# loro-dev/loro

Hardware: AMD Instinct MI355X
Metric: merged docs/sec (batch of N docs x M remote ops) (higher is better)
Workload: dtype u32; 1 GPU; configs[1]: 10000 docs/GPU x 100000-op automerge-paper-shaped text trace, 2 concurrent peers, 3 FastUpdates blobs/doc (4683 op runs, 30 changes, 103435 blob bytes/doc); docs_per_gpu=10000, ops_per_doc=100000, contexts_in_flight=2, streams_per_context=2

## Files before the change

loro_amd/csrc/lm_k_decode.h:

```cpp
#pragma once
#include "lm_dev_util.h"

namespace lm {

struct Dev {
  const uint8_t* data;
  const uint64_t* blob_off;
  const uint32_t* blob_len;
  const uint32_t* doc_blob;
  uint32_t n_blobs, n_docs;
  uint32_t span;
  const uint32_t* res_old_blobs;
  uint32_t loc_cleared;
  uint32_t* posdel;
  const uint64_t* posdel_off;
  uint32_t* pd_row_idx;
  const uint8_t* vvo;
  const uint64_t* vvo_off;
  const uint8_t* doc_fused;
  uint32_t n_op_rows;
  uint32_t* blk_kind;
  uint32_t posdel_redo;
  uint32_t no_linear;
  uint32_t res_vis;
  const uint8_t* front;
  const uint64_t* front_off;
  const uint8_t* froot;
  const uint64_t* froot_off;
  int32_t* blob_status;
  uint32_t* blob_hash;
  uint32_t* blob_nblk;
  uint32_t* blob_blk0;
  uint32_t* blob_doc;
  uint32_t n_blocks;
  BlockDesc* blk;
  uint32_t* bcnt;
  uint32_t* boff;
  ChangeRow* chg;
  uint32_t* dep_peer;
  uint32_t* dep_ctr;
  uint32_t* dep_ci;
  OpRow* op;
  uint64_t* op_val;
  uint32_t* op_blk;
  uint64_t* key_off;
  uint32_t* key_len;
  uint32_t* cid_raw;
  uint32_t* cid_map;
  uint64_t* peer_raw;
  uint32_t* peer_map;
  DocMeta* doc;
  const uint32_t* doc_order;
  uint64_t* peer_uniq;
  uint32_t* peer_end;
  uint32_t* peer_ext;
  uint32_t* peer_base;
  uint32_t* peer_end_all;
  uint32_t* elem_base;
  uint32_t* elem_cap;
  uint32_t* peer_chg0;
  uint32_t* peer_chg1;
  ContRow* cont;
  uint32_t* chg_sorted;
  uint32_t* chg_lamport;
  uint32_t* chg_skip;
  uint32_t* chg_flag;
  uint32_t* chg_mask;
  uint32_t* node_first;
  uint32_t* node_last;
  uint32_t* node_order;
  uint32_t* vvh;
  uint32_t* cp;
  uint32_t* loc;
  uint32_t* dcnt;
  uint8_t* tb;
  uint32_t* it;
  uint8_t* lf_chunk;
  uint32_t* dir_out;
  uint32_t* cont_root0;
  uint32_t* cont_nroot;
  unsigned long long* ht_key;
  unsigned long long* ht_best;
  unsigned long long* ht_pfx;
  uint64_t* ht0;
  uint32_t* ht_cap;
  uint32_t* ht_list;
  uint32_t* ht_cnt;
  unsigned long long* prof;
  uint32_t* fuse;
  uint32_t* dec_stat;
  uint32_t dec_slot;
  uint32_t vs_row_cost;
  uint32_t cut_min_rows;
  uint8_t* out;
  uint64_t* out_off;
  uint8_t* vv_out;
  uint64_t* vv_off;
};
static constexpr int BCN = 8;
enum { BC_CHG = 0, BC_DEP, BC_OP, BC_KEY, BC_CID, BC_PEER, BC_MAPOP, BC_ATOMS };
static constexpr uint32_t VIS_CAP = 1024;
static constexpr uint32_t TB_WIDE = 0xFF, TB_ANCHOR = 0xFE;
static constexpr uint32_t CP_ANCHOR = 0x80000000u, CP_ALIVE = 0x40000000u;

static constexpr uint64_t BIG_BLOB = 32768;
static constexpr uint32_t HASH_G = 4;
LM_DEV uint32_t xx_round(uint32_t v, uint32_t m) { return rotl32(v + m, 13) * 0x9E3779B1u; }
LM_KERNEL LM_WAVES_PER_SIMD(2) LM_ONE_WAVE_GROUPS void k_hash_big_blobs(Dev d, const uint32_t* big, uint32_t n_big) {
  const uint32_t P1 = 0x9E3779B1u, P2 = 0x85EBCA77u, P3 = 0xC2B2AE3Du, P4 = 0x27D4EB2Fu, P5 = 0x165667B1u;
  const uint32_t seed = 0x4f524f4cu;
  uint32_t lane = (uint32_t)lmw::lane(), row = lane >> 4, rl = lane & 15, a = lane & 3;
  uint32_t i = (uint32_t)lmw::bid() * HASH_G + row;
  bool have = i < n_big;
  uint32_t b = big[have ? i : 0u];
  uint64_t blen = have ? d.blob_len[b] : 0ull;
  uint64_t len = blen >= 1024 + 20 ? blen - 20 : 0ull;
  const uint8_t* p = d.data + d.blob_off[b] + 20;
  const uint32_t* w = (const uint32_t*)p + rl;
  uint32_t v = a == 0 ? seed + P1 + P2 : a == 1 ? seed + P2 : a == 2 ? seed : seed - P1;
  const uint32_t n_str = (uint32_t)(len >> 4), n_kb = n_str >> 6;
  const uint32_t T = lmw::reduce_max(n_kb);
  uint32_t xa[16], xb[16], xc[16];
  const uint32_t kb_last = n_kb ? n_kb - 1 : 0u;
#define LM_HASH_LOAD(x, t) do { const uint32_t* q_ = w + (size_t)256 * ((t) < kb_last ? (t) : kb_last); _Pragma("unroll") for (int k_ = 0; k_ < 16; k_++) x[k_] = q_[16 * k_]; } while (0)
#define LM_HASH_CHAIN(x, t) do { uint32_t nv_ = v; _Pragma("unroll") for (int k_ = 0; k_ < 16; k_++) { const uint32_t m_ = x[k_] * P2; \
      nv_ = xx_round(nv_, m_); nv_ = xx_round(nv_, lmw::row_down<4>(m_)); nv_ = xx_round(nv_, lmw::row_down<8>(m_)); nv_ = xx_round(nv_, lmw::row_down<12>(m_)); LM_SCHED_FENCE(); } \
    if ((t) < n_kb) v = nv_; } while (0)
  LM_HASH_LOAD(xa, 0u); LM_HASH_LOAD(xb, 1u);
#pragma unroll 1
  for (uint32_t t = 0; t < T; t += 3) {
    LM_HASH_LOAD(xc, t + 2); LM_HASH_CHAIN(xa, t);
    LM_HASH_LOAD(xa, t + 3); LM_HASH_CHAIN(xb, t + 1);
    LM_HASH_LOAD(xb, t + 4); LM_HASH_CHAIN(xc, t + 2);
  }
#undef LM_HASH_LOAD
#undef LM_HASH_CHAIN
  {
    const uint32_t s0 = n_kb << 6;
#pragma unroll 1
    for (uint32_t c = 0; c < 16; c++) {
      const uint32_t s_ = s0 + 4 * c;
      const uint32_t st_ = s_ + (rl >> 2), stc_ = st_ < n_str ? st_ : (n_str ? n_str - 1 : 0u);
      const uint32_t x = ((const uint32_t*)p)[(size_t)4 * stc_ + a];
      const uint32_t m_ = x * P2;
      uint32_t nv = xx_round(v, m_);
      if (s_ < n_str) v = nv;
      nv = xx_round(v, lmw::row_down<4>(m_));
      if (s_ + 1 < n_str) v = nv;
      nv = xx_round(v, lmw::row_down<8>(m_));
      if (s_ + 2 < n_str) v = nv;
      nv = xx_round(v, lmw::row_down<12>(m_));
      if (s_ + 3 < n_str) v = nv;
    }
  }
  int g0 = (int)(lane & ~15u);
  uint32_t v1 = lmw::shfl(v, g0), v2 = lmw::shfl(v, g0 + 1), v3 = lmw::shfl(v, g0 + 2), v4 = lmw::shfl(v, g0 + 3);
  uint32_t h = rotl32(v1, 1) + rotl32(v2, 7) + rotl32(v3, 12) + rotl32(v4, 18);
  h += (uint32_t)len;
  const uint8_t* q = p + ((uint64_t)n_str << 4);
  const uint8_t* end = p + len;
  while (q + 4 <= end) { h = rotl32(h + ld32le(q) * P3, 17) * P4; q += 4; }
  while (q < end) { h = rotl32(h + (*q) * P5, 11) * P1; q++; }
  h ^= h >> 15; h *= P2; h ^= h >> 13; h *= P3; h ^= h >> 16;
  if (have && rl == 0) d.blob_hash[b] = len >= 16 ? h : 0u;
}

LM_KERNEL void k_frame_count(Dev d) {
  uint32_t b = (uint32_t)(lmw::bid() * lmw::bdim() + lmw::tid());
  if (b >= d.n_blobs) return;
  const uint8_t* p = d.data + d.blob_off[b];
  uint64_t len = d.blob_len[b];
  int32_t st = ST_OK;
  uint32_t nblk = 0;
  if (len < 22) st = ST_DECODE_ERROR;
  else if (!(p[0] == 'l' && p[1] == 'o' && p[2] == 'r' && p[3] == 'o')) st = ST_DECODE_ERROR;
  else {
    uint32_t mode = ((uint32_t)p[20] << 8) | p[21];
    if (mode == 3) st = ST_UNSUPPORTED;
    else if (mode != 4) st = ST_DECODE_ERROR;
    else {
      uint32_t expect = ld32le(p + 16);
      uint32_t h = len >= BIG_BLOB ? d.blob_hash[b] : xxh32_lane(p + 20, len - 20, 0x4f524f4cu);
      if (h != expect) st = ST_CHECKSUM_MISMATCH;
      else {
        Rd r = rd_make(p + 22, len - 22);
        while (r.p < r.end && !r.bad) {
          uint64_t bl = rd_uleb(r);
          if (bl == 0 || bl > rd_left(r)) { r.bad = true; break; }
          r.p += bl;
          nblk++;
        }
        if (r.bad) { st = ST_DECODE_ERROR; nblk = 0; }
      }
    }
  }
  d.blob_status[b] = st;
  d.blob_nblk[b] = nblk;
}

LM_KERNEL void k_frame_fill(Dev d) {
  uint32_t b = (uint32_t)(lmw::bid() * lmw::bdim() + lmw::tid());
  if (b >= d.n_blobs) return;
  if (d.blob_status[b] != ST_OK) return;
  uint64_t base = d.blob_off[b];
  const uint8_t* p = d.data + base;
  uint64_t len = d.blob_len[b];
  Rd r = rd_make(p + 22, len - 22);
  uint32_t bi = d.blob_blk0[b];
  uint32_t nblk = d.blob_nblk[b];
  uint32_t doc = d.blob_doc[b];
  for (uint32_t k = 0; k < nblk; k++, bi++) {
    uint64_t bl = rd_uleb(r);
    BlockDesc* o = d.blk + bi;
    o->base = (uint64_t)(r.p - d.data);
    o->blob = b;
    o->doc = doc;
    o->pad = (uint32_t)bl;
    r.p += bl;
  }
}
LM_KERNEL void k_block_desc(Dev d) {
  uint32_t bi = (uint32_t)(lmw::bid() * lmw::bdim() + lmw::tid());
  if (bi >= d.n_blocks) return;
  BlockDesc bd = d.blk[bi];
  const uint8_t* p0 = d.data + bd.base;
  Rd q = rd_make(p0, bd.pad);
// ... 553 lines not shown
```

loro_amd/csrc/lm_k_integrate_span.h:

```cpp
#pragma once
#include "lm_k_integrate.h"

namespace lm {

static constexpr uint32_t SP_REC = 320;
LM_DEV uint32_t sa_make(uint32_t leaf, uint32_t n, bool nf) { return leaf | (nf ? DIR_NF : 0u) | (n << 18); }
LM_DEV uint32_t sa_leaf(uint32_t a) { return a & DIR_LEAF_MASK; }
LM_DEV uint32_t sa_n(uint32_t a) { return (a >> 18) & 0x7f; }
LM_DEV bool sa_nf(uint32_t a) { return (a & DIR_NF) != 0; }

struct SpanRegs { uint32_t n, id, len, ol, orr, st; };
struct SpanItem { uint32_t id, len, ol, orr, st; };

struct Ts {
  uint32_t* it;
  uint32_t* loc;
  const uint32_t* ebase;
  const uint32_t* cur;
  const uint32_t* end;
  uint32_t* da;
  uint32_t* db;
  uint32_t* ds;
  bool ds_on;
  uint32_t n_dir, dir_cap, n_leaf, leaf_cap, tot_active;
  uint32_t n_alive;
  uint32_t cache_leaf;
  uint32_t cache_p;
  uint32_t cache_pre;
  SpanRegs cr;
  bool dirty;
  uint32_t loc_pend;
  int32_t err;
  uint32_t beyond;
#ifdef LM_PROF
  mutable uint64_t prof[PF_N];
#endif
};
static constexpr int32_t ST_POSDEL = 101;
static constexpr uint32_t PD_CAP = 63;
static constexpr uint32_t PD_LDS = 12;
LM_DEV uint32_t* pd_w(const Ts& t) { return const_cast<uint32_t*>(t.ebase) - PD_LDS; }
template <bool POS>
LM_DEV void pd_stop(Ts& t, uint32_t k, uint32_t left, uint32_t first, uint32_t matched) {
#ifdef LM_EMU_TRACE
  if (getenv("LM_EMU_BASE") && lmw::lane() == 0 && t.err) fprintf(stderr, "pd_stop<%d> with err %d\n", (int)POS, (int)t.err);
#endif
  if (!POS || t.err != ST_RETRY) t.err = ST_POSDEL;
  if (POS && lmw::lane() == 0) { uint32_t* w = pd_w(t); w[0] = k; w[1] = left; w[2] = first; w[3] = matched; }
}

LM_DEV uint32_t ts_g(const Ts& t, uint32_t pid) { return t.ebase[pid_peer(pid)] + pid_ctr(pid); }
LM_DEV bool sp_has(uint32_t id0, uint32_t len, uint32_t x) { return x >= id0 && x - id0 < len; }

LM_DEV SpanRegs sp_load(const Ts& t, uint32_t L, uint32_t n) {
  int lane = lmw::lane();
  lmw::wave_sync();
  if (L == t.cache_leaf) return t.cr;
  PROF_CNT(t, PF_NEXTRA, 1);
  SpanRegs r;
  r.n = n;
  bool in = (uint32_t)lane < n;
  const uint32_t* rec = t.it + (uint64_t)L * SP_REC;
  r.id = in ? rec[lane] : NONE;
  r.len = in ? rec[64 + lane] : 0u;
  r.ol = in ? rec[128 + lane] : NONE;
  r.orr = in ? rec[192 + lane] : NONE;
  r.st = in ? rec[256 + lane] : ST_FUT;
  return r;
}
LM_DEV void sp_write(Ts& t, uint32_t L, const SpanRegs& R) {
  int lane = lmw::lane();
  if ((uint32_t)lane < R.n) {
    uint32_t* rec = t.it + (uint64_t)L * SP_REC;
    rec[lane] = R.id; rec[64 + lane] = R.len; rec[128 + lane] = R.ol; rec[192 + lane] = R.orr; rec[256 + lane] = R.st;
  }
}
LM_DEV uint32_t sp_alen(const SpanRegs& R) { return st_active(R.st) ? R.len : 0u; }
LM_DEV bool sp_nf(const SpanRegs& R) { return lmw::ballot(!(R.st & ST_FUT)) != 0; }
LM_DEV uint64_t sp_hit(const SpanRegs& R, uint32_t x) { return lmw::ballot(x - R.id < R.len); }
#ifndef LM_LOC_SHORT
#define LM_LOC_SHORT 16
#endif
static constexpr uint32_t LOC_SHORT = LM_LOC_SHORT;
#if !defined(LM_LOC_FULL) && !defined(LM_LOC16)
#define LM_LOC16 1
#endif
#ifdef LM_LOC16
#ifndef LM_LOC_W
#define LM_LOC_W 64
#endif
static constexpr uint32_t LOC_W = LM_LOC_W;
LM_DEV void sp_set_loc_lanes(Ts& t, const SpanRegs& R, bool pend, uint32_t L) {
  if (!t.loc) return;
  uint32_t len = pend ? R.len : 0u;
  uint32_t c0 = pid_ctr(R.id);
  uint32_t g = pend ? t.ebase[pid_peer(R.id)] + c0 : 0u;
  if (pend) t.loc[g] = L;
  uint32_t k = LOC_W - (c0 & (LOC_W - 1));
  for (uint32_t i = 0; i < 4 && lmw::any(k < len); i++, k += LOC_W) if (k < len) t.loc[g + k] = L;
  uint64_t m = lmw::ballot(k < len);
  while (m) {
    int j = lmw::ffs64(m);
    m &= m - 1;
    uint32_t gj = lmw::bcast(g, j), lj = lmw::bcast(len, j), kj = lmw::bcast(k, j);
    for (uint32_t kk = kj + LOC_W * (uint32_t)lmw::lane(); kk < lj; kk += 64 * LOC_W) t.loc[gj + kk] = L;
  }
}
LM_DEV uint32_t ts_loc_find(const Ts& t, uint32_t pid) {
  if (!t.loc) return NONE;
  uint32_t ctr = pid_ctr(pid), lo = ctr & ~(LOC_W - 1), eb = t.ebase[pid_peer(pid)];
  uint32_t lane = (uint32_t)lmw::lane();
  uint32_t v = (lane < LOC_W && lo + lane <= ctr) ? t.loc[eb + lo + lane] : NONE;
  uint64_t m = lmw::ballot(v != NONE);
  if (!m) return NONE;
  int top = 63 - __builtin_clzll((unsigned long long)m);
  return lmw::bcast(v, top);
}
#else
LM_DEV void sp_set_loc_lanes(Ts& t, const SpanRegs& R, bool pend, uint32_t L) {
  uint32_t len = pend ? R.len : 0u;
  uint32_t g = pend ? t.ebase[pid_peer(R.id)] + pid_ctr(R.id) : 0u;
  uint32_t lim = len < LOC_SHORT ? len : LOC_SHORT;
  for (uint32_t k = 0; k < lim; k++) t.loc[g + k] = L;
  uint64_t m = lmw::ballot(len > LOC_SHORT);
  while (m) {
    int j = lmw::ffs64(m);
    m &= m - 1;
    uint32_t gj = lmw::bcast(g, j), lj = lmw::bcast(len, j);
    for (uint32_t k = LOC_SHORT + (uint32_t)lmw::lane(); k < lj; k += 64) t.loc[gj + k] = L;
  }
}
#endif
LM_DEV void sp_flush(Ts& t) {
  if (t.cache_leaf == NONE) return;
  if (t.dirty) { sp_write(t, t.cache_leaf, t.cr); t.dirty = false; }
  if (lmw::any(t.loc_pend != 0)) { sp_set_loc_lanes(t, t.cr, t.loc_pend != 0, t.cache_leaf); t.loc_pend = 0; }
}
LM_DEV void sp_flush_loc(Ts& t) {
  if (t.cache_leaf != NONE && lmw::any(t.loc_pend != 0)) { sp_set_loc_lanes(t, t.cr, t.loc_pend != 0, t.cache_leaf); t.loc_pend = 0; }
}
LM_DEV void sd_sync_cached(Ts& t);
LM_DEV void sp_take(Ts& t, uint32_t L) {
  if (t.cache_leaf != L) { sp_flush(t); sd_sync_cached(t); t.cache_leaf = L; t.dirty = false; t.loc_pend = 0; }
}

#ifndef LM_SD_LINEAR
#define LM_SD_LINEAR 128
#endif
static constexpr uint32_t SD_LINEAR = LM_SD_LINEAR;
#ifndef LM_SD_BSH
#define LM_SD_BSH 6
#endif
static constexpr uint32_t SD_BSH = LM_SD_BSH, SD_BS = 1u << LM_SD_BSH;
LM_DEV void sd_block_sum(Ts& t, uint32_t j) {
  uint32_t i = (j << SD_BSH) + (uint32_t)lmw::lane();
  lmw::wave_sync();
  uint32_t s = lmw::reduce_add(((uint32_t)lmw::lane() < SD_BS && i < t.n_dir) ? t.db[i] : 0u);
  if (lmw::lane() == 0) t.ds[j] = s;
  lmw::wave_sync();
}
LM_DEV void sd_sums_from(Ts& t, uint32_t j0) { for (uint32_t j = j0; (j << SD_BSH) < t.n_dir; j++) sd_block_sum(t, j); }
LM_DEV void sd_sync_cached(Ts& t) { if (t.ds_on && t.cache_leaf != NONE && t.cache_p < t.n_dir) sd_block_sum(t, t.cache_p >> SD_BSH); }
LM_DEV void sd_set(Ts& t, uint32_t p, uint32_t a, uint32_t b) {
  lmw::wave_sync();
  uint32_t old = t.db[p];
  lmw::wave_sync();
  if (lmw::lane() == 0) { t.da[p] = a; t.db[p] = b; if (t.ds_on) t.ds[p >> SD_BSH] += b - old; }
  t.tot_active += b - old;
  lmw::wave_sync();
}
LM_DEV void sd_insert_after(Ts& t, uint32_t p, uint32_t a, uint32_t b) {
  int lane = lmw::lane();
  if (t.n_dir >= t.dir_cap) { LM_SETERR(t.err, ST_RETRY); return; }
  lmw::wave_sync();
  uint32_t q = p + 1;
  for (uint32_t hi = t.n_dir; hi > q;) {
    uint32_t c0 = hi > q + 64 ? hi - 64 : q;
    uint32_t i = c0 + (uint32_t)lane;
    bool in = i < hi;
    uint32_t va = in ? t.da[i] : 0u, vb = in ? t.db[i] : 0u;
    lmw::wave_sync();
    if (in) { t.da[i + 1] = va; t.db[i + 1] = vb; }
    lmw::wave_sync();
    hi = c0;
  }
  if (lane == 0) { t.da[q] = a; t.db[q] = b; }
  t.n_dir++;
  t.tot_active += b;
  if (t.cache_leaf != NONE && t.cache_p >= q) t.cache_p++;
  lmw::wave_sync();
  if (!t.ds_on && t.n_dir > SD_LINEAR) { t.ds_on = true; sd_sums_from(t, 0); }
  else if (t.ds_on) sd_sums_from(t, q >> SD_BSH);
}
LM_DEV uint32_t sd_find_kth(Ts& t, uint32_t& k) {
  int lane = lmw::lane();
  lmw::wave_sync();
  uint32_t first = 0;
  if (t.ds_on) {
    sd_sync_cached(t);
    uint32_t nb = (t.n_dir + SD_BS - 1) >> SD_BSH, blk = NONE;
    for (uint32_t j0 = 0; j0 < nb && blk == NONE; j0 += 64) {
      uint32_t j = j0 + (uint32_t)lane;
      uint32_t a = j < nb ? t.ds[j] : 0u;
      uint32_t inc = lmw::scan_incl_add(a);
      uint64_t m = lmw::ballot(inc >= k);
      if (m) { int s2 = lmw::ffs64(m); k -= lmw::bcast(inc, s2) - lmw::bcast(a, s2); blk = j0 + (uint32_t)s2; }
      else k -= lmw::bcast(inc, 63);
    }
    if (blk == NONE) return NONE;
    first = blk << SD_BSH;
  }
  for (uint32_t i0 = first; i0 < t.n_dir; i0 += 64) {
    uint32_t i = i0 + (uint32_t)lane;
    uint32_t a = i < t.n_dir ? t.db[i] : 0u;
    uint32_t inc = lmw::scan_incl_add(a);
    uint64_t m = lmw::ballot(inc >= k);
    if (m) {
      int s = lmw::ffs64(m);
      k -= lmw::bcast(inc, s) - lmw::bcast(a, s);
      return i0 + (uint32_t)s;
    }
    k -= lmw::bcast(inc, 63);
  }
  return NONE;
}
LM_DEV uint32_t sd_find_leaf(const Ts& t, uint32_t L) {
  int lane = lmw::lane();
  lmw::wave_sync();
  for (uint32_t i0 = 0; i0 < t.n_dir; i0 += 64) {
    uint32_t i = i0 + (uint32_t)lane;
    uint64_t m = lmw::ballot(i < t.n_dir && sa_leaf(t.da[i]) == L);
    if (m) return i0 + (uint32_t)lmw::ffs64(m);
  }
  return NONE;
}
LM_DEV uint32_t sd_prefix(Ts& t, uint32_t p) {
  int lane = lmw::lane();
  lmw::wave_sync();
  uint32_t acc = 0, first = 0;
  if (t.ds_on) {
    sd_sync_cached(t);
    uint32_t nbp = p >> SD_BSH;
    for (uint32_t j = (uint32_t)lane; j < nbp; j += 64) acc += t.ds[j];
    first = nbp << SD_BSH;
  }
  for (uint32_t i0 = first; i0 < p; i0 += 64) {
    uint32_t i = i0 + (uint32_t)lane;
    acc += i < p ? t.db[i] : 0u;
  }
  return lmw::reduce_add(acc);
}
LM_DEV bool ts_del_pos_ok(Ts& t, const SpanRegs& R, uint32_t slot, uint32_t s_off, uint32_t st0, uint32_t hint_k) {
  if (t.cache_pre == NONE) t.cache_pre = sd_prefix(t, t.cache_p);
  uint32_t al = sp_alen(R);
  uint32_t inc = lmw::scan_incl_add(al);
  uint32_t before = lmw::bcast(inc, (int)slot) - lmw::bcast(al, (int)slot);
  return st_active(st0) && t.cache_pre + before + s_off + 1 == hint_k;
}
LM_DEV void sd_refresh(Ts& t, uint32_t p, uint32_t L, const SpanRegs& R) {
  sd_set(t, p, sa_make(L, R.n, sp_nf(R)), lmw::reduce_add(sp_alen(R)));
}

LM_DEV SpanRegs sp_shift_in(const SpanRegs& R, uint32_t& lp, uint32_t idx, const SpanItem& A, const SpanItem& B, uint32_t cnt, bool setA, bool setB) {
  uint32_t lane = (uint32_t)lmw::lane();
  SpanRegs N;
  N.n = R.n + cnt;
// ... 830 lines not shown
    U4* c4 = (U4*)dcnt;
    const U4 zero4 = {0, 0, 0, 0};
    for (uint32_t i = (uint32_t)lane; i < (m.atoms + 3) / 4; i += 64) c4[i] = zero4;
  }
  lmw::mem_fence();
  lmw::wave_sync();
  for (uint32_t i0 = 0; i0 < m.n_op; i0 += 64) {
    uint32_t i = i0 + (uint32_t)lane;
    uint32_t g0 = 0, n = 0;
    if (i < m.n_op) {
      const OpRow& r = d.op[m.op0 + i];
      uint32_t ck = r.cidx_kind;
      if ((ck & 0xffff) == cidx && ((ck >> 16) & 0xff) == OK_DEL && (d.chg_flag[r.chg] & 1u)) {
        const ChangeRow& ch = d.chg[r.chg];
        uint32_t peer = ch.peer;
        uint32_t lo = ch.ctr + d.chg_skip[r.chg], hi = ts_vs_target(vv, ov_peer, ov, peer);
        if (lo < r.ctr) lo = r.ctr;
        if (hi > r.ctr + r.len) hi = r.ctr + r.len;
        if (lo < hi && r.a0 < P) {
          uint32_t a = lo - r.ctr, b = hi - r.ctr;
          uint32_t Ln = (uint32_t)(r.a2 < 0 ? -r.a2 : r.a2);
          uint32_t t0, t1;
          if (r.a2 > 0) { t0 = r.a1 + a; t1 = r.a1 + b; }
          else { t0 = r.a1 + (Ln - b); t1 = r.a1 + (Ln - a); }
          uint32_t e = t.end[r.a0];
          if (t1 > e) t1 = e;
          if (t0 < t1 && b <= Ln) { g0 = t.ebase[r.a0] + t0; n = t1 - t0; }
        }
      }
    }
    for (uint32_t k = 0; k < n && k < 16; k++) lmw::atomic_add(&dcnt[g0 + k], 1u);
    uint64_t lm_ = lmw::ballot(n > 16);
    while (lm_) {
      int src = lmw::ffs64(lm_);
      lm_ &= lm_ - 1;
      uint32_t bg = lmw::bcast(g0, src), bn = lmw::bcast(n, src);
      for (uint32_t k = 16 + (uint32_t)lane; k < bn; k += 64) lmw::atomic_add(&dcnt[bg + k], 1u);
    }
  }
  lmw::mem_fence();
  lmw::wave_sync();
  for (uint32_t q = 0; q < t.n_dir; q++) {
    uint32_t a = lmw::first(t.da[q]);
    uint32_t L = sa_leaf(a), n = sa_n(a);
    uint32_t* rec = t.it + (uint64_t)L * SP_REC;
    bool in = (uint32_t)lane < n;
    uint32_t id = in ? rec[lane] : 0u, ln = in ? rec[64 + lane] : 0u, st = in ? rec[256 + lane] : ST_FUT;
    uint32_t st1 = st;
    bool over = false, ragged = false;
    if (in) {
      uint32_t peer = pid_peer(id), ctr = pid_ctr(id);
      uint32_t cnt = dcnt[t.ebase[peer] + ctr];
      over = cnt > 0x7fffu;
      if (over) cnt = 0x7fffu;
      st1 = (st & ~(ST_FUT | ST_DELMASK)) | (ctr >= ts_vs_target(vv, ov_peer, ov, peer) ? ST_FUT : 0u) | (cnt << 8) | (cnt ? ST_EVER : 0u);
#ifdef LM_EMU_CHECK
      for (uint32_t k = 1; k < ln; k++)
        if (dcnt[t.ebase[peer] + ctr + k] != cnt || ((ctr + k >= ts_vs_target(vv, ov_peer, ov, peer)) != ((st1 & ST_FUT) != 0))) {
          fprintf(stderr, "CHECK version sweep: item %u:%u+%u is not uniform at element %u (count %u vs %u)\n", peer, ctr, ln, k, dcnt[t.ebase[peer] + ctr + k], cnt);
          ragged = true;
        }
#endif
    }
    if (lmw::any(over)) { LM_SETERR(t.err, ST_UNSUPPORTED); return; }
    if (lmw::any(ragged)) { LM_SETERR(t.err, ST_INTERNAL); return; }
    if (!lmw::any(in && st1 != st)) continue;
    if (in && st1 != st) rec[256 + lane] = st1;
    uint32_t act = lmw::reduce_add((in && st_active(st1)) ? ln : 0u);
    bool nf = lmw::ballot(in && !(st1 & ST_FUT)) != 0;
    sd_set(t, q, sa_make(L, n, nf), act);
  }
}
LM_DEV bool ts_sweep_pays(const Ts& t, const DocMeta& m, uint32_t P, const uint32_t* vv, uint32_t ov_peer, uint32_t ov, const uint32_t* s_cur) {
  uint32_t dist = 0;
  for (uint32_t p = (uint32_t)lmw::lane(); p < P; p += 64) { uint32_t c = s_cur[p], g = ts_vs_target(vv, ov_peer, ov, p); dist += c > g ? c - g : g - c; }
  dist = lmw::reduce_add(dist);
#ifdef LM_SWEEP_EAGER
  return dist > 0;
#else
  return dist > 256 && (uint64_t)dist * 16 > (uint64_t)m.atoms / 32 + m.n_op + 40ull * t.n_dir + 2048;
#endif
}
LM_DEV bool ts_sweep_pays_batch(const Ts& t, const Dev& d, const DocMeta& m, uint32_t P, const uint32_t* vv, const uint32_t* s_cur) {
  uint32_t dist = 0, np = 0;
  for (uint32_t p = (uint32_t)lmw::lane(); p < P; p += 64) { uint32_t c = s_cur[p], g = vv[p]; dist += c > g ? c - g : g - c; np += c != g ? 1u : 0u; }
  dist = lmw::reduce_add(dist);
  np = lmw::reduce_add(np);
#ifdef LM_SWEEP_EAGER
  return dist > 0;
#else
  const uint64_t rows = (uint64_t)dist * m.n_op / (m.atoms ? m.atoms : 1u);
  return dist > 16 && rows * d.vs_row_cost > 5ull * m.n_op / 4 + m.atoms / 40 + 60ull * t.n_dir + 600ull * np + 500;
#endif
}
#ifndef LM_BATCH_VSWEEP
#define LM_BATCH_VSWEEP 0
#endif
template <bool ML, bool SWEEP, bool VS, bool POS = false>
LM_DEV void ts_goto(Ts& t, const Dev& d, const DocMeta& m, uint32_t cidx, uint32_t P, const uint32_t* vv, uint32_t* s_cur, uint32_t* s_base,
                    bool& base_on, bool conv, uint32_t* loc_real, uint32_t* dcnt_real) {
  int lane = lmw::lane();
  if (!t.loc) {
    bool mv = false;
    for (uint32_t p = (uint32_t)lane; p < P; p += 64) mv |= s_cur[p] != vv[p];
    if (conv || lmw::any(mv)) ts_build_loc(t, loc_real);
  }
  bool reset = false;
  if (base_on) {
    bool same = true;
    uint32_t back = 0;
    for (uint32_t p = (uint32_t)lane; p < P; p += 64) { uint32_t v = vv[p], c = s_cur[p]; same &= v == s_base[p]; back += c > v ? c - v : 0u; }
    back = lmw::reduce_add(back);
#ifdef LM_SWEEP_EAGER
    reset = !lmw::any(!same) && back > 0;
#else
    reset = !lmw::any(!same) && back > 4 * t.n_dir + 32;
#endif
  }
#ifdef LM_EMU_TRACE
  if (getenv("LM_EMU_BASE") && lane == 0) fprintf(stderr, "BASE cont %u: %s%s (n_dir %u)\n", cidx, reset ? "reset" : "move", conv ? " +convert" : "", t.n_dir);
#endif
  if (reset) ts_reset_to_base(t, s_base);
  else if (VS && !base_on && !conv && dcnt_real && (lmw::block_sync(), ts_sweep_pays_batch(t, d, m, P, vv, s_cur))) ts_sweep_version(t, d, m, cidx, P, vv, NONE, 0, s_cur, dcnt_real);
  else
    for (uint32_t p = 0; p < P && !t.err; p++) {
      uint32_t cur = s_cur[p], tgt = vv[p];
      if (cur > tgt) ts_move_ops<ML, SWEEP, POS>(t, d, m, cidx, p, tgt, cur, -1);
      else if (cur < tgt) ts_move_ops<ML, SWEEP, POS>(t, d, m, cidx, p, cur, tgt, +1);
    }
  lmw::block_sync();
  for (uint32_t p = (uint32_t)lane; p < P; p += 64) { s_cur[p] = vv[p]; if (conv) s_base[p] = vv[p]; }
  if (conv && !t.err) { ts_convert_base(t); base_on = true; }
  lmw::block_sync();
}

#ifdef LM_EMU_CHECK
inline bool ts_check(Ts& t, const char* what, uint32_t row) {
  bool ok = true;
  sp_flush(t);
  lmw::wave_sync();
  if (lmw::lane() == 0) {
    uint32_t tot = 0;
    for (uint32_t q = 0; q < t.n_dir && ok; q++) {
      uint32_t a = t.da[q], L = sa_leaf(a), n = sa_n(a), act = 0;
      bool nf = false;
      const uint32_t* rec = t.it + (uint64_t)L * SP_REC;
      for (uint32_t i = 0; i < n; i++) {
        uint32_t id0 = rec[i], ln = rec[64 + i], st = rec[256 + i];
        if (ln == 0) { fprintf(stderr, "CHECK %s row=%u: dir[%u] leaf %u item %u has length 0\n", what, row, q, L, i); ok = false; }
        if (st_active(st)) act += ln;
        nf |= !(st & ST_FUT);
        for (uint32_t k = 0; k < ln && t.loc; k++) {
#ifdef LM_LOC16
          uint32_t expect = (k == 0 || ((id0 + k) & (LOC_W - 1)) == 0) ? L : NONE;
#else
          uint32_t expect = L;
#endif
          if (t.loc[ts_g(t, id0 + k)] != expect) { fprintf(stderr, "CHECK %s row=%u: loc of %u:%u is %u, item lives in leaf %u\n", what, row, id0 >> 24, (id0 & 0xffffff) + k, t.loc[ts_g(t, id0 + k)], L); ok = false; break; }
        }
      }
      if (act != t.db[q] || nf != sa_nf(a)) { fprintf(stderr, "CHECK %s row=%u: dir[%u] leaf %u active %u (cached %u) nf %d (cached %d)\n", what, row, q, L, act, t.db[q], (int)nf, (int)sa_nf(a)); ok = false; }
      tot += act;
    }
    if (ok && t.ds_on)
      for (uint32_t j = 0; (j << SD_BSH) < t.n_dir && ok; j++) {
        if (t.cache_leaf != NONE && j == (t.cache_p >> SD_BSH)) continue;
        uint32_t sum = 0;
        for (uint32_t q = j << SD_BSH; q < ((j + 1) << SD_BSH) && q < t.n_dir; q++) sum += t.db[q];
        if (sum != t.ds[j]) { fprintf(stderr, "CHECK %s row=%u: block %u sums to %u, cached sum %u\n", what, row, j, sum, t.ds[j]); ok = false; }
      }
    if (ok && tot != t.tot_active) { fprintf(stderr, "CHECK %s row=%u: total active %u, cached %u\n", what, row, tot, t.tot_active); ok = false; }
    if (ok && t.cache_leaf != NONE) {
      if (t.cache_p >= t.n_dir || sa_leaf(t.da[t.cache_p]) != t.cache_leaf) { fprintf(stderr, "CHECK %s row=%u: cached leaf %u is not at directory position %u\n", what, row, t.cache_leaf, t.cache_p); ok = false; }
      uint32_t pre = 0;
      for (uint32_t q = 0; q < t.cache_p && q < t.n_dir; q++) pre += t.db[q];
      if (ok && t.cache_pre != NONE && pre != t.cache_pre) { fprintf(stderr, "CHECK %s row=%u: %u active elements before the cached leaf, cached prefix %u\n", what, row, pre, t.cache_pre); ok = false; }
    }
  }
  return lmw::any(!ok) ? false : true;
}
#define TS_CHECK(what, row) do { if (!t.err && !ts_check(t, what, row)) t.err = ST_INTERNAL; } while (0)
#else
#define TS_CHECK(what, row) do {} while (0)
#endif

}
#include "lm_k_integrate_linear.h"
namespace lm {

struct ResDoc {
  uint64_t tk_off;
  uint32_t pcap, ccap;
  uint32_t reset;
  uint32_t elem_cap;
};
struct DevRes {
  const ResDoc* doc;
  uint32_t* tk;
  const uint32_t* dir_a_prev;
  const uint32_t* dir_b_prev;
  uint32_t* dir_b;
};
static constexpr uint32_t TK_HDR = 12, TK_CW = 8;
LM_DEV uint32_t tk_words(uint32_t pcap, uint32_t ccap) { return TK_HDR + 5 * pcap + ccap * (TK_CW + pcap); }
LM_DEV uint32_t* tk_peers(uint32_t* tk) { return tk + TK_HDR; }
LM_DEV uint32_t* tk_applied(uint32_t* tk, uint32_t pcap) { return tk + TK_HDR + 2 * pcap; }
LM_DEV uint32_t* tk_ebase(uint32_t* tk, uint32_t pcap) { return tk + TK_HDR + 3 * pcap; }
LM_DEV uint32_t* tk_ecap(uint32_t* tk, uint32_t pcap) { return tk + TK_HDR + 4 * pcap; }
LM_DEV uint32_t* tk_cont(uint32_t* tk, uint32_t pcap, uint32_t c) { return tk + TK_HDR + 5 * pcap + c * (TK_CW + pcap); }

#ifndef LM_INTEGRATE_WAVES
#define LM_INTEGRATE_WAVES 5
#endif
#if defined(LM_LOC_FULL) && !defined(LM_LAZY_LOC)
#define LM_LAZY_LOC 0
#endif
#ifndef LM_LAZY_LOC
#define LM_LAZY_LOC 1
#endif
#ifndef LM_BASE_RESET
#define LM_BASE_RESET 1
#endif
template <bool ML, bool PLAIN, bool SWEEP = false, bool RES = false, bool FUSE = false, bool POS = false>
LM_DEV void integrate_span_body(Dev d, DevDag g, uint32_t dir_cap, uint32_t pmax, const OpRow* __restrict__ op_ro,
                                const ChangeRow* __restrict__ chg_ro, const uint32_t* __restrict__ sorted_ro,
                                const uint32_t* __restrict__ skip_ro, const uint32_t* __restrict__ vvh_ro, uint32_t retry_pass,
                                uint32_t* retry_count, DevRes rs = DevRes{}) {
  uint32_t doc = d.doc_order[(uint32_t)lmw::bid()];
  int lane = lmw::lane();
  LM_DYN_SHARED(uint32_t, s_mem);
  uint32_t* s_da = s_mem;
  uint32_t* s_db = s_mem + dir_cap;
  uint32_t* s_ds = s_db + dir_cap;
  uint32_t* s_ebase = s_ds + ((dir_cap >> SD_BSH) + 2) + PD_LDS;
  uint32_t* s_cur = s_ebase + pmax;
  uint32_t* s_end = s_cur + pmax;
  uint32_t* s_tgt = s_end + pmax;
  uint32_t* s_app = s_tgt + pmax;
  uint32_t* s_pmap = s_app + pmax;
  DocMeta m = d.doc[doc];
  if (RES) {
    uint32_t* mw = (uint32_t*)&m;
    for (uint32_t i = 0; i < sizeof(DocMeta) / 4; i++) mw[i] = lmw::first(mw[i]);
  }
  uint64_t elem0 = ((uint64_t)m.elem0_hi << 32) | m.elem0_lo;
  {
    uint32_t fl = m.flags;
    if (RES && (fl & DF_PLAIN) && d.front_off[doc + 1] > d.front_off[doc]) fl &= ~DF_PLAIN;
    if (POS ? ((fl & DF_MOVABLE) != 0 || ((fl & DF_PLAIN) != 0) != PLAIN) : (fl & (DF_MOVABLE | DF_PLAIN)) != ((ML ? DF_MOVABLE : 0u) | (PLAIN ? DF_PLAIN : 0u))) return;
    if (PLAIN && !RES && !POS && ((fl & DF_FUSED) != 0 && d.fuse != nullptr) != FUSE) return;
  }
  (void)SWEEP;
  if (retry_pass && m.status != (POS ? ST_POSDEL : ST_RETRY)) return;
  if (status_fatal(m.status) && !retry_pass) return;
  const bool keep_loc = RES && !ML && !retry_pass && (m.flags & DF_LAYOUT_SAME) != 0;
  {
    struct alignas(16) U4 { uint32_t x, y, z, w; };
    U4* l4 = (U4*)(d.loc + elem0);
    const U4 none4 = {NONE, NONE, NONE, NONE};
    uint32_t from4 = 0;
    if (keep_loc) from4 = lmw::first((rs.tk + rs.doc[doc].tk_off)[6]) / 4;
    if (RES || !d.loc_cleared || retry_pass)
      for (uint32_t i = from4 + (uint32_t)lane; i < (m.atoms + 3) / 4; i += 64) l4[i] = none4;
  }
  if (retry_pass) {
    for (uint32_t c = (uint32_t)lane; c < m.n_cont; c += 64) {
      uint32_t ck = d.cont[m.cid0 + c].kind_root & 0xff;
      if (ck == CK_TEXT || ck == CK_LIST || (ML && ck == CK_MOVABLE)) d.cont[m.cid0 + c].touched = 0;
    }
    lmw::block_sync();
    if (lane == 0) d.doc[doc].status = ST_OK;
    m.status = ST_OK;
    lmw::block_sync();
  }
  if (status_fatal(m.status)) return;
  uint32_t P = m.n_peers;
  for (uint32_t p = (uint32_t)lane; p < P; p += 64) { s_ebase[p] = d.elem_base[m.praw0 + p]; s_end[p] = d.peer_end[m.praw0 + p]; }
  if (POS && !RES) for (uint32_t p = (uint32_t)lane; p < P; p += 64) s_app[p] = d.peer_base[m.praw0 + p];
  uint32_t* tk = nullptr;
  uint32_t tk_pcap = 0, P0 = 0, C0 = 0;
  bool fresh = true, renumber = false;
  const bool to_version = RES && !PLAIN && d.front_off[doc + 1] > d.front_off[doc] && !(m.flags & DF_FRONT_ERR);
  if (RES) {
    ResDoc rd;
    {
      const uint32_t* rw = (const uint32_t*)(rs.doc + doc);
      rd.tk_off = ((uint64_t)lmw::first(rw[1]) << 32) | lmw::first(rw[0]);
      rd.pcap = lmw::first(rw[2]); rd.ccap = lmw::first(rw[3]); rd.reset = lmw::first(rw[4]); rd.elem_cap = lmw::first(rw[5]);
    }
    tk = rs.tk + rd.tk_off;
    tk_pcap = rd.pcap;
    if (P > pmax || P > rd.pcap || m.n_cont > rd.ccap) { if (lane == 0) { LM_SETERR(d.doc[doc].status, ST_INTERNAL); tk[0] = 0; } return; }
    for (uint32_t p = (uint32_t)lane; p < P; p += 64) { s_tgt[p] = d.peer_end[m.praw0 + p]; s_end[p] = d.peer_end_all[m.praw0 + p]; s_app[p] = 0; }
    lmw::block_sync();
    P0 = lmw::first(tk[1]); C0 = lmw::first(tk[2]);
    fresh = rd.reset != 0 || retry_pass != 0 || lmw::first(tk[0]) != 1u || P0 > P || C0 > m.n_cont || P0 > rd.pcap;
    if (!fresh) {
      bool lost = false;
      for (uint32_t q = (uint32_t)lane; q < P0; q += 64) {
        uint64_t id = ((uint64_t)tk_peers(tk)[2 * q + 1] << 32) | tk_peers(tk)[2 * q];
        uint32_t lo = 0, hi = P;
        while (lo < hi) { uint32_t mid = (lo + hi) >> 1; if (d.peer_uniq[m.praw0 + mid] < id) lo = mid + 1; else hi = mid; }
        bool ok = lo < P && d.peer_uniq[m.praw0 + lo] == id;
        s_pmap[q] = ok ? lo : 0u;
        lost |= !ok;
        renumber |= ok && lo != q;
        if (ML && ok && tk_ebase(tk, tk_pcap)[q] != d.elem_base[m.praw0 + lo]) lost = true;
      }
      if (ML && (lmw::first(tk[4]) != m.elem0_lo || lmw::first(tk[5]) != m.elem0_hi)) lost = true;
      fresh = lmw::any(lost);
      renumber = lmw::any(renumber);
      lmw::block_sync();
      if (!fresh) for (uint32_t q = (uint32_t)lane; q < P0; q += 64) s_app[s_pmap[q]] = tk_applied(tk, tk_pcap)[q];
    }
    if (lane == 0) tk[0] = 0;
    if (fresh && !retry_pass && lane == 0) lmw::atomic_add(retry_count + 1, 1u);
  }
  lmw::block_sync();
  uint64_t vvh0 = ((uint64_t)m.vvh0_hi << 32) | m.vvh0_lo;
  Ts t;
  t.it = d.it + (uint64_t)m.leaf0 * SP_REC;
  t.loc = d.loc + elem0;
  t.ebase = s_ebase; t.cur = s_cur; t.end = s_end; t.da = s_da; t.db = s_db; t.ds = s_ds; t.ds_on = false;
  t.dir_cap = dir_cap; t.leaf_cap = m.leaf_cap; t.n_leaf = 0; t.err = 0; t.beyond = 0;
  t.n_alive = 0;
  if (lane == 0) {
    uint64_t pl = 0, ri = 0, pcap = PD_CAP;
    if (POS && d.posdel) {
      const uint64_t p0 = d.posdel_off ? d.posdel_off[doc] : (uint64_t)doc * PD_CAP;
      if (d.posdel_off) pcap = d.posdel_off[doc + 1] - p0;
      pl = (uint64_t)(uintptr_t)(d.posdel + p0 * 3);
      if (d.pd_row_idx && pcap > PD_CAP) ri = (uint64_t)(uintptr_t)d.pd_row_idx;
    }
    uint32_t* w = s_ebase - PD_LDS;
    w[0] = w[1] = w[2] = w[3] = w[4] = 0; w[5] = (uint32_t)pl; w[6] = (uint32_t)(pl >> 32);
    w[7] = (uint32_t)(pcap > 0xffffffffull ? 0xffffffffull : pcap); w[8] = (uint32_t)ri; w[9] = (uint32_t)(ri >> 32); w[10] = w[11] = 0;
  }
#ifdef LM_PROF
  for (int i = 0; i < PF_N; i++) t.prof[i] = 0;
  uint64_t pf_begin = lmw::clock();
#endif
  uint32_t dir_used = 0;
  if (m.leaf_cap > MAX_LEAVES_PER_DOC || (retry_pass && retry_pass != 3u && m.leaf_cap > dir_cap) || P > pmax) { if (lane == 0) LM_SETERR(d.doc[doc].status, ST_UNSUPPORTED); return; }
  if (RES && !fresh) {
    t.n_leaf = lmw::first(tk[3]);
    if (t.n_leaf > t.leaf_cap) { fresh = true; t.n_leaf = 0; }
    for (uint32_t c = 0; c < C0 && !fresh && (!keep_loc || renumber); c++) {
      const uint32_t* rec = tk_cont(tk, tk_pcap, c);
      uint32_t r0 = lmw::first(rec[0]), nr = lmw::first(rec[1]);
      for (uint32_t q = 0; q < nr; q++) {
        uint32_t a = lmw::first(rs.dir_a_prev[m.leaf0 + r0 + q]);
        uint32_t L = sa_leaf(a), n = sa_n(a);
        uint32_t* lr = t.it + (uint64_t)L * SP_REC;
        bool in = (uint32_t)lane < n;
        SpanRegs R;
        R.n = n;
        R.id = in ? lr[lane] : NONE; R.len = in ? lr[64 + lane] : 0u;
        if (renumber) {
          uint32_t ol = in ? lr[128 + lane] : NONE, orr = in ? lr[192 + lane] : NONE;
          if (in) {
            R.id = pid_make(s_pmap[pid_peer(R.id)], pid_ctr(R.id));
            if (ol != NONE) ol = pid_make(s_pmap[pid_peer(ol)], pid_ctr(ol));
            if (orr != NONE) orr = pid_make(s_pmap[pid_peer(orr)], pid_ctr(orr));
            lr[lane] = R.id; lr[128 + lane] = ol; lr[192 + lane] = orr;
          }
        }
        if (!keep_loc) sp_set_loc_lanes(t, R, in, L);
      }
    }
    lmw::mem_fence();
    lmw::block_sync();
  }
  for (uint32_t cidx = 0; cidx < m.n_cont && !t.err; cidx++) {
    uint32_t ckind = d.cont[m.cid0 + cidx].kind_root & 0xff;
    if (ckind != CK_TEXT && ckind != CK_LIST && !(ML && ckind == CK_MOVABLE)) continue;
    const bool resume = RES && !fresh && cidx < C0;
    if (!resume && t.n_leaf >= t.leaf_cap) { LM_SETERR(t.err, ST_INTERNAL); break; }
    lmw::block_sync();
    t.cache_leaf = NONE; t.cr.n = 255; t.cache_pre = NONE; t.dirty = false; t.loc_pend = 0;
    for (uint32_t p = (uint32_t)lane; p < P; p += 64) s_cur[p] = 0;
    if (resume) {
      const uint32_t* rec = tk_cont(tk, tk_pcap, cidx);
      uint32_t r0 = lmw::first(rec[0]), nr = lmw::first(rec[1]);
      if (nr == 0 || nr > dir_cap) { if (nr) t.err = ST_RETRY; else LM_SETERR(t.err, ST_INTERNAL); break; }
      uint32_t act = 0;
      for (uint32_t i = (uint32_t)lane; i < nr; i += 64) { uint32_t b = rs.dir_b_prev[m.leaf0 + r0 + i]; s_da[i] = rs.dir_a_prev[m.leaf0 + r0 + i]; s_db[i] = b; act += b; }
      t.n_dir = nr; t.tot_active = lmw::reduce_add(act); t.n_alive = lmw::first(rec[2]);
      lmw::block_sync();
      t.ds_on = nr > SD_LINEAR;
      if (t.ds_on) sd_sums_from(t, 0);
      for (uint32_t q = (uint32_t)lane; q < P0; q += 64) s_cur[s_pmap[q]] = rec[TK_CW + q];
    } else {
      uint32_t L0 = t.n_leaf++;
      if (lane == 0) { s_da[0] = sa_make(L0, 0, false); s_db[0] = 0; }
      t.n_dir = 1; t.tot_active = 0; t.n_alive = 0; t.ds_on = false;
    }
    lmw::block_sync();
    bool touched = false;
    t.loc = (PLAIN && !RES && LM_LAZY_LOC) ? nullptr : d.loc + elem0;
    bool base_on = false;
    uint32_t* s_base = s_tgt;
    uint32_t oi0 = 0;
    if (PLAIN && !RES && LM_LINEAR && LM_LAZY_LOC && (m.flags & DF_CUT) && !d.no_linear) {
      Tl c;
      tl_none(c);
      bool emptied = false;
      const uint32_t* op_w = (const uint32_t*)op_ro;
      for (; oi0 < m.n_nodes && !t.err; oi0++) {
        uint32_t n = d.node_order[m.chg0 + oi0];
        if (lmw::first(g.node_done[m.chg0 + n]) & 2u) break;
        uint32_t first = d.node_first[m.chg0 + n], last = d.node_last[m.chg0 + n];
        uint32_t node_peer = chg_ro[sorted_ro[m.chg0 + first]].peer;
        const ChangeRow lc = chg_ro[sorted_ro[m.chg0 + last]];
        RowWin w;
        w.base = NONE - 64; w.lim = m.op0 + m.n_op; w.cur = 0; w.nxt = 0;
        bool node_contig = false, node_mine = true;
        if (FUSE && last > first) {
          bool bad = false, mine = false;
          for (uint32_t i = first + (uint32_t)lane; i <= last; i += 64) {
            uint32_t cr0 = sorted_ro[m.chg0 + i];
            if (i < last) { const ChangeRow c0 = chg_ro[cr0], c1 = chg_ro[sorted_ro[m.chg0 + i + 1]]; bad |= c0.op0 + c0.n_op != c1.op0; }
            mine |= ((d.chg_mask[2 * (uint64_t)cr0 + ((cidx >> 5) & 1)] >> (cidx & 31)) & 1) != 0;
          }
          node_contig = !lmw::any(bad);
          if (node_contig) node_mine = lmw::any(mine);
        }
        for (uint32_t ci = first; ci <= last && node_mine && !t.err; ci++) {
          uint32_t crow = sorted_ro[m.chg0 + ci];
          const ChangeRow ch = chg_ro[crow];
          uint32_t n_rows = ((lmw::first(d.chg_mask[2 * (uint64_t)crow + ((cidx >> 5) & 1)]) >> (cidx & 31)) & 1) ? ch.n_op : 0u;
          if (FUSE && node_contig) { n_rows = lc.op0 + lc.n_op - ch.op0; ci = last; }
          struct alignas(16) U4 { uint32_t x, y, z, w; };
          const uint32_t row_end = ch.op0 + n_rows;
          const U4 z4 = {0u, 0u, 0u, 0u};
          U4 na = z4, nb = z4;
          if (ch.op0 + (uint32_t)lane < row_end) { const U4* p = (const U4*)(op_ro + ch.op0 + (uint32_t)lane); na = p[0]; nb = p[1]; }
          for (uint32_t base = ch.op0; base < row_end && !t.err; base += 64) {
            U4 a4 = na, b4 = nb;
            if (base + 64 + (uint32_t)lane < row_end) { const U4* p = (const U4*)(op_ro + base + 64 + (uint32_t)lane); na = p[0]; nb = p[1]; }
            const bool in = base + (uint32_t)lane < row_end;
            if (FUSE && in && (a4.x & OPF_HEAD)) {
              const uint32_t row = base + (uint32_t)lane;
              uint32_t fa1 = d.fuse[2 * (uint64_t)row];
              int32_t fa2 = (int32_t)d.fuse[2 * (uint64_t)row + 1];
              a4.z = (uint32_t)(fa2 < 0 ? -fa2 : fa2);
              if (((a4.x >> 16) & 0xff) == OK_DEL) { b4.y = fa1; b4.z = (uint32_t)fa2; }
            }
            const uint32_t kindv = (a4.x >> 16) & 0xff;
            const bool insv = (kindv == OK_TEXT_INS) | (kindv == OK_LIST_INS), delv = kindv == OK_DEL;
            const int32_t a2v = (int32_t)b4.z;
            const uint32_t Lnv = (uint32_t)(a2v < 0 ? -a2v : a2v);
            const uint32_t badv = (Lnv ^ a4.z) | (a4.y >> 31) | ((b4.z >> 31) & ((a4.y + 1u - Lnv) >> 31));
            uint32_t codev = insv ? 1u : (delv ? (badv ? 3u : 2u) : 0u);
            uint32_t posv = delv ? (a2v > 0 ? a4.y : a4.y + 1u - Lnv) : a4.y;
            uint32_t lenv = delv ? Lnv : a4.z;
            const uint32_t pidv = pid_make(node_peer, a4.w);
            uint64_t mine = lmw::ballot(in & ((a4.x & 0xffff) == cidx) & (!FUSE | !(a4.x & OPF_CONT)) & (codev != 0));
            while (mine && !t.err) {
              const int j = lmw::ffs64(mine);
              mine &= mine - 1;
              const uint32_t code = lmw::bcast(codev, j), pos = lmw::bcast(posv, j), n = lmw::bcast(lenv, j);
              touched = true;
              if (code == 1) tl_insert(t, c, pos, lmw::bcast(pidv, j), n);
              else if (code == 2) {
                const uint32_t left = tl_delete(t, c, pos, n, emptied);
                if (left) { lenv = lane == j ? left : lenv; mine |= 1ull << j; }
              } else LM_SETERR(t.err, ST_DATA_CORRUPTION);
            }
          }
        }
        if (lane == 0) s_cur[node_peer] = lc.ctr + lc.len;
      }
      tl_finish(t, c, emptied);
      lmw::block_sync();
#ifdef LM_EMU_TRACE
// ... 136 lines not shown
          if (POS) last_row = row;
          if (FUSE) {
            if (r.cidx_kind & OPF_HEAD) {
              lmw::wave_sync();
              uint32_t fa1 = lmw::first(d.fuse[2 * (uint64_t)row]);
              int32_t fa2 = (int32_t)lmw::first(d.fuse[2 * (uint64_t)row + 1]);
              r.len = (uint32_t)(fa2 < 0 ? -fa2 : fa2);
              if (((r.cidx_kind >> 16) & 0xff) == OK_DEL) { r.a1 = fa1; r.a2 = fa2; }
            }
          }
          if (!PLAIN && r.ctr + r.len <= skip_to) continue;
          uint32_t kind = (r.cidx_kind >> 16) & 0xff;
          uint32_t a = PLAIN ? 0u : (skip_to > r.ctr ? skip_to - r.ctr : 0);
          touched = true;
          if (!PLAIN && r.ctr + a >= pe) continue;
          uint32_t b = PLAIN ? r.len : (r.ctr + r.len <= pe ? r.len : pe - r.ctr);
          if (!(PLAIN && !RES) && !checked_out) {
            checked_out = true;
            if (!RES) ts_goto<ML, SWEEP, (!ML && !PLAIN && !RES && !POS && LM_BATCH_VSWEEP), POS>(t, d, m, cidx, P, vv, s_cur, s_base, base_on, conv_node, d.loc + elem0, d.dcnt ? d.dcnt + elem0 : nullptr);
            else {
            lmw::block_sync();
            if (RES && !ML && d.dcnt && ts_sweep_pays(t, m, P, vv, node_peer, r.ctr + a, s_cur)) ts_sweep_version(t, d, m, cidx, P, vv, node_peer, r.ctr + a, s_cur, d.dcnt + elem0);
            else
            for (uint32_t p = 0; p < P && !t.err; p++) {
              uint32_t cur = s_cur[p], tgt = vv[p];
              if (RES && p == node_peer) tgt = r.ctr + a;
              if (cur > tgt) ts_move_ops<ML, SWEEP>(t, d, m, cidx, p, tgt, cur, -1);
              else if (cur < tgt) ts_move_ops<ML, SWEEP>(t, d, m, cidx, p, cur, tgt, +1);
            }
            lmw::block_sync();
            for (uint32_t p = (uint32_t)lane; p < P; p += 64) s_cur[p] = (RES && p == node_peer) ? r.ctr + a : vv[p];
            lmw::block_sync();
            }
            PROF_ADD(t, PF_CHECKOUT);
            TS_CHECK("checkout", row);
          }
          PROF_ADD(t, PF_ROW);
          uint32_t mv_to = NONE;
          if (ML && kind == OK_LIST_MOVE) {
            uint32_t tgt = ts_active_id_at(t, (uint32_t)r.a2);
            if (tgt == NONE || (uint32_t)r.prop >= t.tot_active) { LM_SETERR(t.err, ST_DATA_CORRUPTION); break; }
            if (lane == 0) (d.cp + elem0)[ts_g(t, pid_make(node_peer, r.ctr))] = tgt;
            mv_to = (uint32_t)r.prop;
            r.prop = r.a2; r.a0 = pid_peer(tgt); r.a1 = pid_ctr(tgt); r.a2 = 1; kind = OK_DEL;
          }
          for (;;) {
            if (kind == OK_TEXT_INS || kind == OK_LIST_INS) {
              ts_insert<POS>(t, (uint32_t)r.prop + a, pid_make(node_peer, r.ctr + a), b - a);
              TS_CHECK("insert", row);
            } else if (PLAIN || kind == OK_DEL) {
              uint32_t Ln = (uint32_t)(r.a2 < 0 ? -r.a2 : r.a2);
              uint32_t t0, t1;
              if (r.a2 > 0) { t0 = r.a1 + a; t1 = r.a1 + b; }
              else { t0 = r.a1 + (Ln - b); t1 = r.a1 + (Ln - a); }
              const uint32_t not_del = PLAIN ? (kind ^ OK_DEL) : 0u;
              const uint32_t bad_bits = (Ln ^ r.len) | ((uint32_t)r.prop >> 31) | (((uint32_t)r.a2 >> 31) & (((uint32_t)r.prop + 1u - Ln) >> 31));
              uint32_t hint = 0;
              if (a == 0 && b == r.len) hint = r.a2 > 0 ? (uint32_t)r.prop + 1 : (uint32_t)r.prop + 2 - Ln;
              if (not_del | bad_bits) { if (!not_del) LM_SETERR(t.err, ST_DATA_CORRUPTION); t1 = t0; hint = 0; }
              if (POS && !RES && hint && !t.err && t1 > t0 && t1 <= lmw::first(s_app[r.a0])) {
                lmw::wave_sync();
                if (lane == 0) { uint32_t* w = pd_w(t); w[0] = hint; w[1] = t1 - t0; w[2] = pid_make(r.a0, t0); w[3] = 0; }
                ts_del_positional(t, row);
              } else
              ts_update_range<POS>(t, r.a0, t0, t1, UPD_DEL_INC, hint);
              PROF_ADD(t, PF_DELETE);
              PROF_CNT(t, PF_NDEL, 1);
              TS_CHECK("delete", row);
            } else if (!PLAIN && kind == OK_STYLE_START) {
              ts_insert<POS>(t, (uint32_t)r.prop, pid_make(node_peer, r.ctr), 1);
            } else if (!PLAIN && kind == OK_STYLE_END) {
              uint32_t end_pos = NONE;
              if (row > ch.op0) {
                const OpRow pr = op_ro[row - 1];
                if (((pr.cidx_kind >> 16) & 0xff) == OK_STYLE_START && pr.ctr + 1 == r.ctr && (pr.cidx_kind & 0xffff) == cidx)
                  end_pos = (uint32_t)pr.prop + pr.a0;
              }
              if (end_pos == NONE) { LM_SETERR(t.err, ST_UNSUPPORTED); break; }
              uint32_t pos = end_pos + 1 < t.tot_active ? end_pos + 1 : t.tot_active;
              ts_insert<POS>(t, pos, pid_make(node_peer, r.ctr), 1);
            }
            if (!ML || mv_to == NONE || t.err) break;
            r.prop = (int32_t)mv_to; kind = OK_LIST_INS; mv_to = NONE;
          }
          }
        }
        if (POS && t.err == ST_POSDEL) {
          ts_del_positional(t, last_row);
          row0 = last_row + 1;
          goto rows_again;
        }
        }
        if (checked_out && lane == 0) s_cur[node_peer] = (FUSE && node_contig) ? pe : (ch.ctr + ch.len < pe ? ch.ctr + ch.len : pe);
      }
      lmw::block_sync();
    }
    if (RES && !PLAIN && to_version && !t.err) {
      lmw::block_sync();
      if (!ML && d.dcnt && ts_sweep_pays(t, m, P, s_tgt, NONE, 0, s_cur)) ts_sweep_version(t, d, m, cidx, P, s_tgt, NONE, 0, s_cur, d.dcnt + elem0);
      else
      for (uint32_t p = 0; p < P && !t.err; p++) {
        uint32_t cur = s_cur[p], tgt = s_tgt[p];
        if (cur > tgt) ts_move_ops<ML, SWEEP>(t, d, m, cidx, p, tgt, cur, -1);
        else if (cur < tgt) ts_move_ops<ML, SWEEP>(t, d, m, cidx, p, cur, tgt, +1);
      }
      lmw::block_sync();
      for (uint32_t p = (uint32_t)lane; p < P; p += 64) s_cur[p] = s_tgt[p];
      lmw::block_sync();
      TS_CHECK("closing checkout", 0);
      if (t.err) break;
    }
    if (RES) touched = true;
    sp_flush(t);
    lmw::block_sync();
    if (dir_used + t.n_dir > m.leaf_cap) { LM_SETERR(t.err, ST_INTERNAL); break; }
    for (uint32_t i = (uint32_t)lane; i < t.n_dir; i += 64) d.dir_out[m.leaf0 + dir_used + i] = s_da[i];
    if (RES) {
      for (uint32_t i = (uint32_t)lane; i < t.n_dir; i += 64) rs.dir_b[m.leaf0 + dir_used + i] = s_db[i];
      uint32_t* rec = tk_cont(tk, tk_pcap, cidx);
      for (uint32_t p = (uint32_t)lane; p < P; p += 64) rec[TK_CW + p] = s_cur[p];
      if (lane == 0) { rec[0] = dir_used; rec[1] = t.n_dir; rec[2] = t.n_alive; }
    }
    if (lane == 0) {
      d.cont_root0[m.cid0 + cidx] = dir_used;
      d.cont_nroot[m.cid0 + cidx] = t.n_dir;
      if (touched && (t.n_alive > 0 || (RES && !PLAIN && to_version && t.tot_active > 0))) d.cont[m.cid0 + cidx].touched = 1;
    }
    dir_used += t.n_dir;
    lmw::block_sync();
  }
  if (!t.err && t.beyond) t.err = ST_DATA_CORRUPTION;
  if (t.err == ST_POSDEL && RES && !ML && d.posdel_redo && lane == 0) lmw::atomic_or(&d.doc[doc].flags, DF_REDO);
  if (t.err == ST_POSDEL && (POS || RES || ML || !d.posdel)) t.err = ST_DATA_CORRUPTION;
  if (POS && retry_pass == 3u && t.err == ST_RETRY) t.err = ST_POSDEL;
  if (t.err && lane == 0) {
    d.doc[doc].status = t.err;
    if (t.err == ST_RETRY) lmw::atomic_add(retry_count, 1u);
    if (t.err == ST_POSDEL) lmw::atomic_add(retry_count + 3, 1u);
  }
  if (RES && !t.err) {
    for (uint32_t p = (uint32_t)lane; p < P; p += 64) {
      uint64_t id = d.peer_uniq[m.praw0 + p];
      tk_peers(tk)[2 * p] = (uint32_t)id; tk_peers(tk)[2 * p + 1] = (uint32_t)(id >> 32);
      tk_applied(tk, tk_pcap)[p] = s_end[p];
      tk_ebase(tk, tk_pcap)[p] = s_ebase[p];
      tk_ecap(tk, tk_pcap)[p] = d.elem_cap[m.praw0 + p];
    }
    for (uint32_t c = (uint32_t)lane; c < m.n_cont; c += 64) {
      uint32_t ck = d.cont[m.cid0 + c].kind_root & 0xff;
      if (ck != CK_TEXT && ck != CK_LIST && !(ML && ck == CK_MOVABLE)) { uint32_t* rec = tk_cont(tk, tk_pcap, c); rec[0] = 0; rec[1] = 0; rec[2] = 0; }
    }
    lmw::mem_fence();
    lmw::block_sync();
    if (lane == 0) { tk[1] = P; tk[2] = m.n_cont; tk[3] = t.n_leaf; tk[4] = m.elem0_lo; tk[5] = m.elem0_hi; tk[6] = (m.atoms + 3) & ~3u; tk[7] = m.pending_lo | m.pending_hi; tk[8] = m.atoms; tk[0] = 1; }
  }
  if (lane == 0) d.doc[doc].pad0 = dir_used;
#ifdef LM_PROF
  t.prof[PF_TOTAL] = lmw::clock() - pf_begin;
  if (lane == 0) for (int i = 0; i < PF_N; i++) d.prof[(uint64_t)doc * PF_N + i] = t.prof[i];
#endif
}
LM_KERNEL LM_WAVES_PER_SIMD(LM_INTEGRATE_WAVES) void k_integrate_span(Dev d, DevDag g, uint32_t dir_cap, uint32_t pmax, const OpRow* __restrict__ op_ro,
                                const ChangeRow* __restrict__ chg_ro, const uint32_t* __restrict__ sorted_ro,
                                const uint32_t* __restrict__ skip_ro, const uint32_t* __restrict__ vvh_ro, uint32_t retry_pass,
                                uint32_t* retry_count) {
  integrate_span_body<false, false>(d, g, dir_cap, pmax, op_ro, chg_ro, sorted_ro, skip_ro, vvh_ro, retry_pass, retry_count);
}
LM_KERNEL LM_WAVES_PER_SIMD(LM_INTEGRATE_WAVES) void k_integrate_span_plain(Dev d, DevDag g, uint32_t dir_cap, uint32_t pmax, const OpRow* __restrict__ op_ro,
                                const ChangeRow* __restrict__ chg_ro, const uint32_t* __restrict__ sorted_ro,
                                const uint32_t* __restrict__ skip_ro, const uint32_t* __restrict__ vvh_ro, uint32_t retry_pass,
                                uint32_t* retry_count) {
  integrate_span_body<false, true>(d, g, dir_cap, pmax, op_ro, chg_ro, sorted_ro, skip_ro, vvh_ro, retry_pass, retry_count);
}
LM_KERNEL LM_WAVES_PER_SIMD(LM_INTEGRATE_WAVES) void k_integrate_span_plain_sweep(Dev d, DevDag g, uint32_t dir_cap, uint32_t pmax, const OpRow* __restrict__ op_ro,
                                const ChangeRow* __restrict__ chg_ro, const uint32_t* __restrict__ sorted_ro,
                                const uint32_t* __restrict__ skip_ro, const uint32_t* __restrict__ vvh_ro, uint32_t retry_pass,
                                uint32_t* retry_count) {
  integrate_span_body<false, true, true>(d, g, dir_cap, pmax, op_ro, chg_ro, sorted_ro, skip_ro, vvh_ro, retry_pass, retry_count);
}
LM_KERNEL LM_WAVES_PER_SIMD(LM_INTEGRATE_WAVES) void k_integrate_span_plain_fuse(Dev d, DevDag g, uint32_t dir_cap, uint32_t pmax, const OpRow* __restrict__ op_ro,
                                const ChangeRow* __restrict__ chg_ro, const uint32_t* __restrict__ sorted_ro,
                                const uint32_t* __restrict__ skip_ro, const uint32_t* __restrict__ vvh_ro, uint32_t retry_pass,
                                uint32_t* retry_count) {
  integrate_span_body<false, true, true, false, true>(d, g, dir_cap, pmax, op_ro, chg_ro, sorted_ro, skip_ro, vvh_ro, retry_pass, retry_count);
}
LM_KERNEL LM_WAVES_PER_SIMD(LM_INTEGRATE_WAVES) void k_integrate_span_ml(Dev d, DevDag g, uint32_t dir_cap, uint32_t pmax, const OpRow* __restrict__ op_ro,
                                const ChangeRow* __restrict__ chg_ro, const uint32_t* __restrict__ sorted_ro,
                                const uint32_t* __restrict__ skip_ro, const uint32_t* __restrict__ vvh_ro, uint32_t retry_pass,
                                uint32_t* retry_count) {
  integrate_span_body<true, false>(d, g, dir_cap, pmax, op_ro, chg_ro, sorted_ro, skip_ro, vvh_ro, retry_pass, retry_count);
}
LM_KERNEL LM_WAVES_PER_SIMD(4) LM_ONE_WAVE_GROUPS void k_integrate_span_pos(Dev d, DevDag g, uint32_t dir_cap, uint32_t pmax, const OpRow* __restrict__ op_ro,
                                const ChangeRow* __restrict__ chg_ro, const uint32_t* __restrict__ sorted_ro,
                                const uint32_t* __restrict__ skip_ro, const uint32_t* __restrict__ vvh_ro, uint32_t retry_pass,
                                uint32_t* retry_count) {
  integrate_span_body<false, false, false, false, false, true>(d, g, dir_cap, pmax, op_ro, chg_ro, sorted_ro, skip_ro, vvh_ro, retry_pass, retry_count);
}
LM_KERNEL LM_WAVES_PER_SIMD(4) LM_ONE_WAVE_GROUPS void k_integrate_span_pos_plain(Dev d, DevDag g, uint32_t dir_cap, uint32_t pmax, const OpRow* __restrict__ op_ro,
                                const ChangeRow* __restrict__ chg_ro, const uint32_t* __restrict__ sorted_ro,
                                const uint32_t* __restrict__ skip_ro, const uint32_t* __restrict__ vvh_ro, uint32_t retry_pass,
                                uint32_t* retry_count) {
  integrate_span_body<false, true, true, false, false, true>(d, g, dir_cap, pmax, op_ro, chg_ro, sorted_ro, skip_ro, vvh_ro, retry_pass, retry_count);
}
#ifndef LM_RES_WAVES
#define LM_RES_WAVES 4
#endif
LM_KERNEL LM_WAVES_PER_SIMD(LM_RES_WAVES) LM_ONE_WAVE_GROUPS void k_integrate_span_res(Dev d, DevDag g, uint32_t dir_cap, uint32_t pmax, const OpRow* __restrict__ op_ro,
                                const ChangeRow* __restrict__ chg_ro, const uint32_t* __restrict__ sorted_ro,
                                const uint32_t* __restrict__ skip_ro, const uint32_t* __restrict__ vvh_ro, uint32_t retry_pass,
                                uint32_t* retry_count, DevRes rs) {
  integrate_span_body<false, false, true, true>(d, g, dir_cap, pmax, op_ro, chg_ro, sorted_ro, skip_ro, vvh_ro, retry_pass, retry_count, rs);
}
#ifndef LM_RES_PLAIN_WAVES
#define LM_RES_PLAIN_WAVES LM_INTEGRATE_WAVES
#endif
LM_KERNEL LM_WAVES_PER_SIMD(LM_RES_PLAIN_WAVES) LM_ONE_WAVE_GROUPS void k_integrate_span_res_plain(Dev d, DevDag g, uint32_t dir_cap, uint32_t pmax, const OpRow* __restrict__ op_ro,
                                const ChangeRow* __restrict__ chg_ro, const uint32_t* __restrict__ sorted_ro,
                                const uint32_t* __restrict__ skip_ro, const uint32_t* __restrict__ vvh_ro, uint32_t retry_pass,
                                uint32_t* retry_count, DevRes rs) {
  integrate_span_body<false, true, true, true>(d, g, dir_cap, pmax, op_ro, chg_ro, sorted_ro, skip_ro, vvh_ro, retry_pass, retry_count, rs);
}
LM_KERNEL LM_WAVES_PER_SIMD(LM_RES_WAVES) LM_ONE_WAVE_GROUPS void k_integrate_span_res_ml(Dev d, DevDag g, uint32_t dir_cap, uint32_t pmax, const OpRow* __restrict__ op_ro,
                                const ChangeRow* __restrict__ chg_ro, const uint32_t* __restrict__ sorted_ro,
                                const uint32_t* __restrict__ skip_ro, const uint32_t* __restrict__ vvh_ro, uint32_t retry_pass,
                                uint32_t* retry_count, DevRes rs) {
  integrate_span_body<true, false, true, true>(d, g, dir_cap, pmax, op_ro, chg_ro, sorted_ro, skip_ro, vvh_ro, retry_pass, retry_count, rs);
}

LM_KERNEL void k_res_layout(Dev d, DevRes rs) {
  uint32_t doc = (uint32_t)lmw::bid();
  int lane = lmw::lane();
  LM_SHARED(uint32_t, s_base, MAX_PEERS);
  LM_SHARED(uint32_t, s_cap, MAX_PEERS);
  const DocMeta m = d.doc[doc];
  if (status_fatal(m.status)) return;
  const ResDoc rd = rs.doc[doc];
  uint32_t* tk = rs.tk + rd.tk_off;
  const uint32_t P = m.n_peers;
  if (P > MAX_PEERS) return;
  for (uint32_t p = (uint32_t)lane; p < P; p += 64) { s_base[p] = NONE; s_cap[p] = 0; }
  lmw::block_sync();
  bool same = !rd.reset && tk[0] == 1u && tk[4] == m.elem0_lo && tk[5] == m.elem0_hi && tk[1] <= P && tk[1] <= rd.pcap &&
              tk[2] <= m.n_cont && tk[3] <= m.leaf_cap;
  uint32_t top = 0;
  if (same) {
    uint32_t P0 = tk[1];
    bool bad = false;
    for (uint32_t q = (uint32_t)lane; q < P0; q += 64) {
      uint64_t id = ((uint64_t)tk_peers(tk)[2 * q + 1] << 32) | tk_peers(tk)[2 * q];
      uint32_t lo = 0, hi = P;
      while (lo < hi) { uint32_t mid = (lo + hi) >> 1; if (d.peer_uniq[m.praw0 + mid] < id) lo = mid + 1; else hi = mid; }
      if (lo < P && d.peer_uniq[m.praw0 + lo] == id && d.peer_ext[m.praw0 + lo] <= tk_ecap(tk, rd.pcap)[q]) { s_base[lo] = tk_ebase(tk, rd.pcap)[q]; s_cap[lo] = tk_ecap(tk, rd.pcap)[q]; }
      else bad = true;
    }
    same = !lmw::any(bad);
    top = tk[8];
  }
  lmw::block_sync();
  if (!same) { top = 0; for (uint32_t p = (uint32_t)lane; p < P; p += 64) s_base[p] = NONE; }
  lmw::block_sync();
  for (uint32_t p0 = 0; p0 < P; p0 += 64) {
    uint32_t p = p0 + (uint32_t)lane;
    bool need = p < P && s_base[p] == NONE;
    uint32_t ext = p < P ? d.peer_ext[m.praw0 + p] : 0u;
    uint32_t cap = need ? ((ext + ext / 2 + 64 + 3) & ~3u) : 0u;
    uint32_t inc = lmw::scan_incl_add(cap);
    if (need) { s_base[p] = top + inc - cap; s_cap[p] = cap; }
    top += lmw::bcast(inc, 63);
  }
  lmw::block_sync();
  if (top > rd.elem_cap) {
    if (same) {
      same = false; top = 0;
      for (uint32_t p0 = 0; p0 < P; p0 += 64) {
        uint32_t p = p0 + (uint32_t)lane;
        uint32_t ext = p < P ? d.peer_ext[m.praw0 + p] : 0u;
        uint32_t cap = p < P ? ((ext + ext / 2 + 64 + 3) & ~3u) : 0u;
        uint32_t inc = lmw::scan_incl_add(cap);
        if (p < P) { s_base[p] = top + inc - cap; s_cap[p] = cap; }
        top += lmw::bcast(inc, 63);
      }
      lmw::block_sync();
    }
    if (top > rd.elem_cap) { if (lane == 0) LM_SETERR(d.doc[doc].status, ST_INTERNAL); return; }
  }
  for (uint32_t p = (uint32_t)lane; p < P; p += 64) { d.elem_base[m.praw0 + p] = s_base[p]; d.elem_cap[m.praw0 + p] = s_cap[p]; }
  if (lane == 0) {
    uint32_t fl = d.doc[doc].flags & ~(DF_LAYOUT_SAME | DF_FILL_KEPT);
    if (same) fl |= DF_LAYOUT_SAME | (tk[7] == 0u ? DF_FILL_KEPT : 0u);
    d.doc[doc].flags = fl;
    d.doc[doc].atoms = top;
  }
}

LM_KERNEL void k_cont_untouch(Dev d, uint32_t n_cid) {
  uint32_t t = (uint32_t)(lmw::bid() * lmw::bdim() + lmw::tid());
  if (t < n_cid) d.cont[t].touched = 0;
}
LM_KERNEL void k_res_exists(Dev d, DevRes rs, uint32_t mode) {
  uint32_t doc = (uint32_t)lmw::bid();
  int lane = lmw::lane();
  const DocMeta m = d.doc[doc];
  if (status_fatal(m.status)) return;
  const ResDoc rd = rs.doc[doc];
  if (m.n_cont > rd.ccap) return;
  uint32_t* tk = rs.tk + rd.tk_off;
  for (uint32_t c = (uint32_t)lane; c < m.n_cont; c += 64) {
    uint32_t* rec = tk_cont(tk, rd.pcap, c);
    uint32_t t = d.cont[m.cid0 + c].touched ? 1u : 0u;
    uint32_t e = mode == 1 ? t : ((mode == 2 ? rec[4] == 1u : rec[3] == 1u) ? 1u : 0u) | t;
    rec[3] = e;
    if (mode == 1) rec[4] = e;
    d.cont[m.cid0 + c].touched = e;
  }
}

}
```

loro_amd/csrc/lm_k_scan.h:

```cpp
#pragma once
#include "lm_wave.h"

namespace lm {

static constexpr int SCAN_TILE = 256;

LM_KERNEL void k_scan_tile(const uint32_t* in, uint32_t* out, uint32_t* tile_sum, uint32_t n, uint32_t ncomp) {
  LM_SHARED(uint32_t, s_w, 4);
  uint32_t tile = (uint32_t)lmw::bid();
  uint32_t row = tile * SCAN_TILE + (uint32_t)lmw::tid();
  int lane = lmw::lane(), w = lmw::wave_in_block();
  for (uint32_t c = 0; c < ncomp; c++) {
    uint32_t v = row < n ? in[(uint64_t)row * ncomp + c] : 0;
    uint32_t inc = lmw::scan_incl_add(v);
    if (lane == 63) s_w[w] = inc;
    lmw::block_sync();
    uint32_t base = 0;
    for (int k = 0; k < w; k++) base += s_w[k];
    if (row < n) out[(uint64_t)row * ncomp + c] = base + inc - v;
    if (lmw::tid() == SCAN_TILE - 1) tile_sum[(uint64_t)tile * ncomp + c] = base + inc;
    lmw::block_sync();
  }
}
LM_KERNEL void k_scan_sums(uint32_t* tile_sum, uint32_t n_tiles, uint32_t ncomp, uint32_t* totals) {
  int lane = lmw::lane();
  for (uint32_t c = 0; c < ncomp; c++) {
    uint32_t run = 0;
    for (uint32_t t0 = 0; t0 < n_tiles; t0 += 64) {
      uint32_t t = t0 + (uint32_t)lane;
      uint32_t v = t < n_tiles ? tile_sum[(uint64_t)t * ncomp + c] : 0;
      uint32_t inc = lmw::scan_incl_add(v);
      if (t < n_tiles) tile_sum[(uint64_t)t * ncomp + c] = run + inc - v;
      run += lmw::bcast(inc, 63);
    }
    if (lane == 0) totals[c] = run;
  }
}
LM_KERNEL void k_scan_add(uint32_t* out, const uint32_t* tile_sum, const uint32_t* totals, uint32_t n, uint32_t ncomp) {
  uint32_t tile = (uint32_t)lmw::bid();
  uint32_t row = tile * SCAN_TILE + (uint32_t)lmw::tid();
  for (uint32_t c = 0; c < ncomp; c++) {
    if (row < n) out[(uint64_t)row * ncomp + c] += tile_sum[(uint64_t)tile * ncomp + c];
    if (row == n) out[(uint64_t)row * ncomp + c] = totals[c];
  }
}

LM_KERNEL void k_selftest(uint32_t* out, uint32_t rounds) {
  LM_SHARED(uint32_t, s_in, 64);
  LM_SHARED(uint64_t, s_in64, 64);
  int lane = lmw::lane();
  uint32_t bad = 0;
  uint32_t x = 0x9E3779B9u * (uint32_t)(lane + 1) + (uint32_t)lmw::bid();
  for (uint32_t r = 0; r < rounds; r++) {
    x ^= x << 13; x ^= x >> 17; x ^= x << 5;
    uint32_t v = (r & 1) ? (x & 0xffff) : (x % 65u);
    uint32_t a = lmw::scan_incl_add(v), b = lmw::scan_incl_add_shfl(v);
    bad += a != b ? 1u : 0u;
    uint64_t m = lmw::ballot((v & 1) != 0);
    uint32_t c = (uint32_t)lmw::popc64(m & ((2ull << lane) - 1));
    uint32_t dref = lmw::scan_incl_add_shfl(v & 1);
    bad += c != dref ? 1u : 0u;
    uint32_t s1 = lmw::shift_up(x, 1), s2 = lmw::shift_up(x, 2), r1 = lmw::shfl_up(x, 1), r2 = lmw::shfl_up(x, 2);
    bad += s1 != r1 ? 1u : 0u;
    bad += s2 != r2 ? 1u : 0u;

    uint32_t w;
    switch (r & 3u) {
      case 0: w = x; break;
      case 1: w = 0x9E3779B9u * (r + 1u) + (uint32_t)lmw::bid(); break;
      case 2: w = 0u; break;
      default: w = (x & 0x10u) ? (x | 0x80000000u) : 0u; break;
    }
    const uint64_t w64 = ((uint64_t)x << 32) | (uint64_t)(w ^ 0xA5A5A5A5u);
    const int src = (lane * 7 + (int)r) & 63;
    lmw::block_sync();
    s_in[lane] = w; s_in64[lane] = w64;
    lmw::block_sync();
    uint32_t e_add = 0, e_max = 0, e_rmax = 0, e_rmin = 0xffffffffu, e_radd = 0;
    for (int i = 0; i < 64; i++) {
      uint32_t t = s_in[i];
      if (i <= lane) { e_add += t; e_max = t > e_max ? t : e_max; }
      e_radd += t; e_rmax = t > e_rmax ? t : e_rmax; e_rmin = t < e_rmin ? t : e_rmin;
    }
    bad += lmw::scan_incl_add(w) != e_add ? 1u : 0u;
    bad += lmw::scan_incl_max(w) != e_max ? 1u : 0u;
    bad += lmw::reduce_add(w) != e_radd ? 1u : 0u;
    bad += lmw::reduce_max(w) != e_rmax ? 1u : 0u;
    bad += lmw::reduce_min(w) != e_rmin ? 1u : 0u;
    bad += lmw::shift_up(w, 1) != (lane >= 1 ? s_in[lane - 1] : w) ? 1u : 0u;
    bad += lmw::shift_up(w, 2) != (lane >= 2 ? s_in[lane - 2] : w) ? 1u : 0u;
    bad += lmw::shift_up0(w, 1) != (lane >= 1 ? s_in[lane - 1] : 0u) ? 1u : 0u;
    bad += lmw::shift_up0(w, 2) != (lane >= 2 ? s_in[lane - 2] : 0u) ? 1u : 0u;
    bad += lmw::row_down<4>(w) != ((lane & 15) + 4 > 15 ? 0u : s_in[lane + 4]) ? 1u : 0u;
    bad += lmw::row_down<8>(w) != ((lane & 15) + 8 > 15 ? 0u : s_in[lane + 8]) ? 1u : 0u;
    bad += lmw::row_down<12>(w) != ((lane & 15) + 12 > 15 ? 0u : s_in[lane + 12]) ? 1u : 0u;
    bad += lmw::shfl64(w64, src) != s_in64[src] ? 1u : 0u;
    bad += lmw::first(w) != s_in[0] ? 1u : 0u;
  }
  lmw::block_sync();
  s_in[lane] = bad;
  lmw::block_sync();
  if (lane == 0) { uint32_t tot = 0; for (int i = 0; i < 64; i++) tot += s_in[i]; out[lmw::bid()] = tot; }
}

LM_KERNEL void k_fill_words(uint32_t* p, uint64_t n4, uint32_t v, uint32_t n_threads) {
  struct alignas(16) U4 { uint32_t x, y, z, w; };
  U4* q = (U4*)p;
  const U4 w4 = {v, v, v, v};
  for (uint64_t i = (uint64_t)lmw::bid() * (uint64_t)lmw::bdim() + (uint64_t)lmw::tid(); i < n4; i += n_threads) q[i] = w4;
}

}
```

loro_amd/csrc/lm_pipeline.h:

```cpp
#pragma once
#include <algorithm>
#include <map>
#include <mutex>
#include <thread>
#include <atomic>
#include <cstdint>
#include <cstring>
#include <cstdlib>
#include <string>
#include <vector>
#include <stdexcept>
#include "lm_k_scan.h"
#include "lm_k_emit.h"
#include "lm_k_lww_doc.h"
#include "lm_k_map_fused.h"
#include "lm_k_fuse.h"
#include "lm_k_lca.h"
#include "lm_k_richtext.h"
#include "lm_k_cursor.h"
#include "lm_k_delta.h"
#include "lm_snapshot.h"
#include "lm_export.h"
#include "lm_snapshot_base.h"

namespace lm {

struct DBuf {
  void* p = nullptr;
  size_t cap = 0;
  void ensure(size_t n) {
    if (n <= cap) return;
    if (p) lmbe::dfree(p);
    size_t want = n + n / 8 + 256;
    p = lmbe::dalloc(want);
    if (!p) throw std::runtime_error("device allocation failed");
    cap = want;
  }
  void ensure_keep(size_t n, size_t keep) {
    if (n <= cap) return;
    size_t want = n + n / 2 + 256;
    void* q = lmbe::dalloc(want);
    if (!q) throw std::runtime_error("device allocation failed");
    if (p && keep) { lmbe::d2d(q, p, keep < cap ? keep : cap); lmbe::sync(); }
    if (p) lmbe::dfree(p);
    p = q;
    cap = want;
  }
  void release() { if (p) lmbe::dfree(p); p = nullptr; cap = 0; }
  template <class T> T* as() { return (T*)p; }
};

struct DocResult {
  int32_t status;
  uint64_t json_off, json_len, vv_off, vv_len, pending;
  uint64_t json_xxh64;
};

struct KernelTime { std::string name; double ms; };

struct HostRegions {
  std::mutex mu;
  std::map<const uint8_t*, size_t> r;
  void add(const void* p, size_t n) { std::lock_guard<std::mutex> g(mu); r[(const uint8_t*)p] = n; }
  bool remove(const void* p) { std::lock_guard<std::mutex> g(mu); return r.erase((const uint8_t*)p) != 0; }
  const uint8_t* find(const uint8_t* p, size_t n, size_t* bytes) {
    std::lock_guard<std::mutex> g(mu);
    auto it = r.upper_bound(p);
    if (it == r.begin()) return nullptr;
    --it;
    if (p < it->first || (size_t)(p - it->first) + n > it->second) return nullptr;
    if (bytes) *bytes = it->second;
    return it->first;
  }
};
inline HostRegions& host_regions() { static HostRegions h; return h; }

struct Engine {
  uint32_t n_docs = 0, n_blobs = 0;
  uint64_t data_bytes = 0, in_bytes = 0;
  std::vector<uint64_t> h_blob_off, h_front_off, h_froot_off;
  std::vector<uint8_t> h_front_bytes;
  std::vector<uint8_t> h_froot;
  std::vector<uint32_t> h_blob_len, h_doc_blob, h_blob_doc;
  DBuf b_data, b_blob_off, b_blob_len, b_doc_blob, b_blob_doc, b_front, b_front_off, b_froot, b_froot_off, b_blob_hash, b_big;
  DBuf b_blob_status, b_blob_nblk, b_blob_blk0, b_tile, b_tot;
  DBuf b_blk, b_bcnt, b_boff, b_blk_kind, b_doc_fused, b_mf_docs, b_mf_key0;
  std::vector<uint8_t> h_fused;
  uint32_t n_fused = 0;
  DBuf b_chg, b_dep_peer, b_dep_ctr, b_dep_ci, b_op, b_op_val, b_op_blk, b_key_off, b_key_len, b_cid_raw, b_cid_map, b_peer_raw, b_peer_map;
  DBuf b_doc, b_peer_uniq, b_peer_end, b_peer_ext, b_peer_base, b_peer_end_all, b_elem_base, b_peer_chg0, b_peer_chg1, b_cont;
  DBuf b_chg_mask, b_chg_sorted, b_chg_lamport, b_chg_skip, b_chg_flag, b_node_first, b_node_last, b_node_order, b_vvh;
  DBuf b_blk_sorted, b_chg_node, b_node_done, b_node_lam;
  DBuf b_cp, b_loc, b_tb, b_fuse, b_dcnt, b_posdel;
  DBuf b_it, b_dir_out, b_lf_chunk;
  DBuf b_cont_root0, b_cont_nroot;
  DBuf b_ht_key, b_ht_pfx, b_ht_best, b_ht0, b_ht_cap, b_ht_list, b_ht_cnt;
  DBuf b_out, b_out_off, b_vv_out, b_vv_off, b_hash, b_order, b_prof, b_slab, b_vslab, b_slab_off, b_vslab_off, b_slab2, b_slab2_off;
  uint64_t payload_bytes = 0;
  std::vector<uint64_t> h_prof, h_hash, h_ht0;
  std::vector<uint32_t> h_ht_cap, h_ht_full;
  std::vector<DocMeta> h_doc;
  std::vector<DocResult> results;
  std::vector<uint8_t> h_out, h_vv;
  std::vector<uint64_t> h_out_off, h_vv_off;
  uint64_t out_bytes = 0, vv_bytes = 0;
  bool ran = false, fetched = false;
  Dev last_d;
  DBuf b_rt_out, b_rt_off, b_rt_len;
  std::vector<uint8_t> h_rt;
  std::vector<uint64_t> h_rt_off;
  std::vector<uint32_t> h_rt_len;
  std::vector<int32_t> h_rt_status;
  bool rt_ran = false;
  int rt_launches = 0;
  DBuf b_cur_doc, b_cur_dg, b_cur_grp, b_cur_q, b_cur_names, b_cur_res;
  bool keep_tombstones = false;
  double cur_ms = 0;
  DBuf b_dl_q, b_dl_bnd, b_dl_bits, b_dl_res, b_dl_out, b_dl_off, b_dl_pack, b_dl_poff;
  uint64_t dl_d2h_bytes = 0;
  std::vector<KernelTime> dl_times;
  int dl_launches = 0;
  std::vector<KernelTime> times;
  bool profiling = false;
  std::string last_error;
  uint64_t device_bytes = 0;
  uint32_t last_retries = 0, last_reemits = 0, last_posdel = 0;
  lmbe::StreamCtx* sc = nullptr;
  long long* sum_rows = nullptr;
  long long sum_id0 = 0, sum_stride = 1;

  struct BlobRef { uint64_t off; uint32_t len; };
  bool resident = false;
  uint32_t shared_mode = 0;
  std::vector<std::vector<BlobRef>> r_blobs;
  std::vector<uint32_t> r_step;
  std::vector<std::vector<uint8_t>> r_front;
  uint64_t arena_top = 0;
  bool tables_valid = false;
  std::vector<uint32_t> tk_leaf0, tk_leaf_cap, tk_pcap, tk_ccap, tk_elem_cap, h_old_blobs;
  std::vector<uint64_t> tk_off, tk_elem0;
  uint64_t elem_top = 0;
  DBuf b_elem_cap, b_old_blobs, b_prev_doc, b_prev_uniq, b_prev_end, b_lca_out, b_lca_scratch, b_lca_off;
  bool have_prev = false;
  std::vector<uint32_t> h_lca;
  std::vector<uint8_t> tk_reset;
  void upload_res() {
    std::vector<ResDoc> hres(n_docs);
    for (uint32_t i = 0; i < n_docs; i++) hres[i] = ResDoc{tk_off[i], tk_pcap[i], tk_ccap[i], tk_reset[i], tk_elem_cap[i]};
    b_res.ensure((size_t)n_docs * sizeof(ResDoc));
    lmbe::h2d(b_res.p, hres.data(), (size_t)n_docs * sizeof(ResDoc));
  }
  uint64_t tk_top = 0;
  uint32_t leaf_top = 0;
  int dir_parity = 0;
  DBuf b_tk, b_res, b_dir_out2, b_dir_b, b_dir_b2, b_doc_saved;
  uint32_t last_fresh = 0;
  struct Saved {
    Dev d; DevDag g;
    uint32_t NB = 0, NC = 0, NO = 0, NCID = 0, NP = 0, dir_cap = 0, dir_opt = 0, pmax = 0;
    uint64_t ht = 0;
    bool any_ml = false, any_common = false;
    std::vector<DocMeta> h_doc;
  } sv;

  struct Knobs { bool span = true, decode_wave = true, no_opt_dir = false, loc_memset = true; int plain = 2; uint32_t dec_slot = 1264, dec_slot_big = 4096, dec_big_mode = 1, dir_opt_max = 0; size_t lds_pad = 0; long long slab_cap = -1; uint32_t ht_opt = 2048, cut_min_rows = 2048, vs_row_cost = 300; bool lww_lds = true, fuse_rows = true, version_sweep = true, span_auto = true, linear = true, posdel = true, reclass = true, redo = true, map_fused = true, snapshot_state = true, snapshot_state_force = false, stage_direct = true; uint32_t mf_min_rows = 2048, mf_chg_ratio = 4, pd_state_pieces = 2; } kn;
  void read_knobs() {
    Knobs k;
    if (const char* e = getenv("LM_SPAN")) k.span = atoi(e) != 0;
    if (const char* e = getenv("LM_PLAIN")) k.plain = atoi(e);
    if (const char* e = getenv("LM_DECODE")) k.decode_wave = atoi(e) != 0;
    if (const char* e = getenv("LM_RECLASS")) k.reclass = atoi(e) != 0;
    if (const char* e = getenv("LM_DEC_SLOT")) k.dec_slot = ((uint32_t)atoi(e) + 15u) & ~15u;
    if (const char* e = getenv("LM_DEC_SLOT_BIG")) k.dec_slot_big = ((uint32_t)atoi(e) + 15u) & ~15u;
    if (const char* e = getenv("LM_DEC_BIG_MODE")) k.dec_big_mode = (uint32_t)atoi(e);
    if (const char* e = getenv("LM_LDS_PAD")) k.lds_pad = (size_t)atoi(e);
    k.no_opt_dir = getenv("LM_NO_OPT_DIR") != nullptr;
    if (const char* e = getenv("LM_LOC_MEMSET")) k.loc_memset = atoi(e) != 0;
    if (const char* e = getenv("LM_DIR_OPT_MAX")) k.dir_opt_max = (uint32_t)atoi(e);
    if (const char* e = getenv("LM_SLAB_CAP")) k.slab_cap = atoll(e);
    if (const char* e = getenv("LM_HT_OPT")) k.ht_opt = (uint32_t)atoi(e);
    if (const char* e = getenv("LM_CUT_MIN_ROWS")) k.cut_min_rows = (uint32_t)atoll(e);
    if (const char* e = getenv("LM_SPAN_AUTO")) k.span_auto = atoi(e) != 0;
    if (const char* e = getenv("LM_VS_ROW_COST")) k.vs_row_cost = (uint32_t)atoi(e);
    if (const char* e = getenv("LM_VERSION_SWEEP")) k.version_sweep = atoi(e) != 0;
    if (const char* e = getenv("LM_FUSE_ROWS")) k.fuse_rows = atoi(e) != 0;
    if (const char* e = getenv("LM_POSDEL")) k.posdel = atoi(e) != 0;
    if (const char* e = getenv("LM_LINEAR")) k.linear = atoi(e) != 0;
    if (const char* e = getenv("LM_LWW_LDS")) k.lww_lds = atoi(e) != 0;
    if (const char* e = getenv("LM_REDO")) k.redo = atoi(e) != 0;
    if (const char* e = getenv("LM_MAP_FUSED")) k.map_fused = atoi(e) != 0;
    if (const char* e = getenv("LM_MF_MIN_ROWS")) k.mf_min_rows = (uint32_t)atoi(e);
    if (const char* e = getenv("LM_STAGE_DIRECT")) k.stage_direct = atoi(e) != 0;
    if (const char* e = getenv("LM_PD_STATE_PIECES")) k.pd_state_pieces = (uint32_t)atoi(e);
    if (const char* e = getenv("LM_SNAPSHOT_STATE")) { k.snapshot_state = atoi(e) != 0; k.snapshot_state_force = atoi(e) == 2; }
    if (const char* e = getenv("LM_MF_CHG_RATIO")) k.mf_chg_ratio = (uint32_t)atoi(e);
    if (force_span) { k.span = true; k.span_auto = false; k.posdel = true; k.redo = false; k.map_fused = false; }
    kn = k;
  }
  bool force_span = false;
  bool allow_state = true;
  std::vector<uint8_t> h_vvo;
  std::vector<uint64_t> h_vvo_off;
  std::vector<std::vector<std::vector<uint8_t>>> st_hist;
  uint32_t n_state_docs = 0;
  bool stage_history_only = false;
  DBuf b_vvo, b_vvo_off, b_pd_off, b_pd_row;
  std::vector<uint8_t> redo_hist;
  bool st_valid = false;
  std::vector<uint32_t> st_doc_blob, st_blob_len;
  std::vector<uint64_t> st_blob_off, st_froot_off;
  std::vector<uint8_t> st_froot;
  std::vector<uint32_t> redo_docs;
  struct RedoItem { uint32_t doc; const uint8_t* front; size_t front_len; };
  bool redo_by_history(uint32_t doc) const { return doc < redo_hist.size() && redo_hist[doc] != 0; }
  void stage_from(const std::vector<Engine*>& parents, const std::vector<RedoItem>& items) {
    for (Engine* pe : parents) if (!pe->st_valid) throw std::runtime_error("redo: the staged blobs are gone");
    std::vector<std::vector<const uint8_t*>> bp(items.size());
    std::vector<std::vector<size_t>> bl(items.size());
    std::vector<DocIn> in(items.size());
    for (size_t k = 0; k < items.size(); k++) {
      const uint32_t i = items[k].doc;
      Engine& parent = *parents[k];
      if (parent.redo_by_history(i)) for (auto& hb : parent.st_hist[i]) { bp[k].push_back(hb.data()); bl[k].push_back(hb.size()); }
      else
      for (uint32_t b = parent.st_doc_blob[i]; b < parent.st_doc_blob[i + 1]; b++) { bp[k].push_back(parent.st_base + parent.st_blob_off[b]); bl[k].push_back(parent.st_blob_len[b]); }
      in[k] = DocIn{bp[k].data(), bl[k].data(), bp[k].size(), items[k].front, items[k].front_len};
    }
    stage_history_only = true;
    try { stage(in.data(), in.size()); } catch (...) { stage_history_only = false; throw; }
    stage_history_only = false;
    h_froot.clear();
    h_froot_off.assign(items.size() + 1, 0);
    for (size_t k = 0; k < items.size(); k++) {
      h_froot_off[k] = h_froot.size();
      const uint32_t i = items[k].doc;
      Engine& parent = *parents[k];
      if ((size_t)i + 1 < parent.st_froot_off.size()) h_froot.insert(h_froot.end(), parent.st_froot.begin() + parent.st_froot_off[i], parent.st_froot.begin() + parent.st_froot_off[i + 1]);
    }
    h_froot_off[items.size()] = h_froot.size();
    h_vvo.clear(); h_vvo_off.assign(items.size() + 1, 0); n_state_docs = 0;
    for (size_t k = 0; k < items.size(); k++) {
      h_vvo_off[k] = h_vvo.size();
      Engine& parent = *parents[k];
      const uint32_t i = items[k].doc;
      if (parent.n_state_docs && (size_t)i + 1 < parent.h_vvo_off.size() && parent.h_vvo_off[i + 1] > parent.h_vvo_off[i] && !parent.redo_by_history(i)) {
        h_vvo.insert(h_vvo.end(), parent.h_vvo.begin() + parent.h_vvo_off[i], parent.h_vvo.begin() + parent.h_vvo_off[i + 1]);
        n_state_docs++;
      }
    }
    h_vvo_off[items.size()] = h_vvo.size();
    lmbe::bind(sc);
    if (n_state_docs) {
      b_vvo.ensure(h_vvo.size() + 16); lmbe::h2d(b_vvo.p, h_vvo.data(), h_vvo.size());
      b_vvo_off.ensure((items.size() + 1) * 8); lmbe::h2d(b_vvo_off.p, h_vvo_off.data(), (items.size() + 1) * 8);
    }
    b_froot.ensure(h_froot.size() + 16); if (!h_froot.empty()) lmbe::h2d(b_froot.p, h_froot.data(), h_froot.size());
    b_froot_off.ensure((items.size() + 1) * 8); lmbe::h2d(b_froot_off.p, h_froot_off.data(), (items.size() + 1) * 8);
    lmbe::sync();
  }

  explicit Engine(int device) { sc = lmbe::stream_create(device); }
  Engine(const Engine&) = delete;
  Engine& operator=(const Engine&) = delete;
  uint8_t* h_stage = nullptr;
  const uint8_t* st_base = nullptr;
  bool staged_direct = false;
  size_t h_stage_cap = 0;
  ~Engine() { release_all(); if (h_stage) lmbe::hfree(h_stage); lmbe::stream_destroy(sc); }
  void release_all() {
    DBuf* all[] = {&b_front, &b_front_off, &b_froot, &b_froot_off, &b_blob_hash, &b_big, &b_data, &b_blob_off, &b_blob_len, &b_doc_blob, &b_blob_doc, &b_blob_status, &b_blob_nblk, &b_blob_blk0, &b_tile, &b_tot,
                   &b_vvo, &b_vvo_off, &b_blk, &b_bcnt, &b_boff, &b_blk_kind, &b_doc_fused, &b_mf_docs, &b_mf_key0, &b_chg, &b_dep_peer, &b_dep_ctr, &b_dep_ci, &b_op, &b_op_val, &b_op_blk, &b_key_off, &b_key_len,
                   &b_cid_raw, &b_cid_map, &b_peer_raw, &b_peer_map, &b_doc, &b_peer_uniq, &b_peer_end, &b_peer_ext, &b_peer_base, &b_peer_end_all, &b_elem_base,
                   &b_peer_chg0, &b_peer_chg1, &b_cont, &b_chg_mask, &b_chg_sorted, &b_chg_lamport, &b_chg_skip, &b_chg_flag, &b_node_first,
                   &b_node_last, &b_node_order, &b_vvh, &b_blk_sorted, &b_chg_node, &b_node_done, &b_node_lam, &b_cp, &b_loc, &b_tb, &b_it,
                   &b_dir_out, &b_lf_chunk, &b_fuse, &b_dcnt, &b_posdel, &b_pd_off, &b_pd_row,
                   &b_cont_root0, &b_cont_nroot, &b_prof, &b_hash, &b_order, &b_ht_key, &b_ht_pfx, &b_ht_best, &b_ht0, &b_ht_cap, &b_ht_list, &b_ht_cnt, &b_slab, &b_vslab, &b_slab_off, &b_vslab_off, &b_slab2, &b_slab2_off, &b_out, &b_out_off,
                   &b_vv_out, &b_vv_off, &b_tk, &b_res, &b_dir_out2, &b_dir_b, &b_dir_b2, &b_doc_saved, &b_elem_cap, &b_old_blobs, &b_prev_doc, &b_prev_uniq, &b_prev_end, &b_lca_out, &b_lca_scratch, &b_lca_off};
    for (DBuf* b : all) b->release();
    for (DBuf* b : {&b_dl_q, &b_dl_bnd, &b_dl_bits, &b_dl_res, &b_dl_out, &b_dl_off, &b_dl_pack, &b_dl_poff}) b->release();
  }

  struct DocIn { const uint8_t* const* blobs; const size_t* lens; size_t n; const uint8_t* front; size_t front_len; uint8_t state_root = 0; };
  void stage(const DocIn* docs, size_t nd) {
    lmbe::bind(sc);
    read_knobs();
    n_docs = (uint32_t)nd;
    h_doc_blob.assign(nd + 1, 0);
    size_t nb = 0;
    for (size_t i = 0; i < nd; i++) { h_doc_blob[i] = (uint32_t)nb; nb += docs[i].n; }
    h_doc_blob[nd] = (uint32_t)nb;
    n_blobs = (uint32_t)nb;
    h_blob_off.assign(nb + 1, 0);
    h_blob_len.assign(nb, 0);
    h_blob_doc.assign(nb, 0);
    uint64_t off = 0;
    in_bytes = 0;
    size_t b = 0;
    std::vector<const uint8_t*> bsrc(nb);
    std::vector<size_t> blen(nb);
    std::vector<std::vector<uint8_t>> conv;
    std::vector<uint8_t>& froot = h_froot;
    froot.clear();
    size_t best_changes = 0;
    bool have_snapshot = false;
    h_froot_off.assign(nd + 1, 0);
    static const uint8_t stub_decode[22] = {'l', 'o', 'r', 'o', 0, 0, 0, 0, 0, 0, 0, 0, 0, 0, 0, 0, 0, 0, 0, 0, 0xff, 0xff};
    static const uint8_t stub_checksum[22] = {'l', 'o', 'r', 'o', 0, 0, 0, 0, 0, 0, 0, 0, 0, 0, 0, 0, 0, 0, 0, 0, 0, 4};
    std::vector<std::vector<uint8_t>> vvo_tmp(nd);
    st_hist.assign(nd, {});
    n_state_docs = 0;
    const bool state_off = stage_history_only;
    auto is_mode = [](const uint8_t* p, size_t l, uint8_t mode) { return l >= 22 && memcmp(p, "loro", 4) == 0 && p[20] == 0 && p[21] == mode; };
    for (size_t i = 0; i < nd; i++) {
      if (docs[i].n >= 2 && !docs[i].front && kn.snapshot_state && allow_state && !state_off) {
        size_t ks = docs[i].n, n3 = 0, n4 = 0;
        for (size_t k = 0; k < docs[i].n; k++) { if (is_mode(docs[i].blobs[k], docs[i].lens[k], 3)) { n3++; ks = k; } else if (is_mode(docs[i].blobs[k], docs[i].lens[k], 4)) n4++; }
        std::vector<uint8_t> o2, vv2, roots2;
        lmsnap::StateBase sb;
        std::vector<std::pair<const uint8_t*, size_t>> U;
        std::vector<std::vector<uint8_t>> outU;
        bool pays = true;
        if (n3 == 1 && n3 + n4 == docs[i].n) for (size_t k = 0; k < docs[i].n; k++) if (k != ks) U.emplace_back(docs[i].blobs[k], docs[i].lens[k]);
        if (n3 == 1 && n3 + n4 == docs[i].n && lmsnap::snapshot_state_to_updates(docs[i].blobs[ks], docs[i].lens[ks], o2, vv2, &roots2, false, &sb) &&
            lmsnap::rebase_updates_on_state(sb, U, outU, &pays) && (pays || kn.snapshot_state_force)) {
          h_froot_off[i] = froot.size();
          froot.insert(froot.end(), roots2.begin(), roots2.end());
          size_t u = 0;
          for (size_t k = 0; k < docs[i].n; k++, b++) {
            if (k == ks) { st_hist[i].emplace_back(docs[i].blobs[ks], docs[i].blobs[ks] + docs[i].lens[ks]); conv.push_back(std::move(o2)); }
            else { st_hist[i].emplace_back(docs[i].blobs[k], docs[i].blobs[k] + docs[i].lens[k]); conv.push_back(std::move(outU[u++])); }
            bsrc[b] = conv.back().data(); blen[b] = conv.back().size();
          }
          vvo_tmp[i].resize(8);
          for (int x = 0; x < 8; x++) vvo_tmp[i][x] = (uint8_t)(sb.synth_peer >> (8 * x));
          vvo_tmp[i].insert(vvo_tmp[i].end(), vv2.begin(), vv2.end());
          n_state_docs++;
          if (const char* dump = getenv("LM_DUMP_STATE_BASE")) {
            for (size_t k = 0; k < docs[i].n; k++) {
              std::string fn = std::string(dump) + std::to_string(i) + "_" + std::to_string(k) + ".bin";
              if (FILE* f = fopen(fn.c_str(), "wb")) { fwrite(bsrc[b - docs[i].n + k], 1, blen[b - docs[i].n + k], f); fclose(f); }
            }
          }
          continue;
        }
      }
      for (size_t k = 0; k < docs[i].n; k++, b++) {
        const uint8_t* p = docs[i].blobs[k];
        size_t l = docs[i].lens[k];
        if (k == 0) h_froot_off[i] = froot.size();
        if (k == 0) { best_changes = 0; have_snapshot = false; }
        if (l >= 22 && memcmp(p, "loro", 4) == 0 && p[20] == 0 && p[21] == 3) {
          if (docs[i].n == 1 && !docs[i].front && kn.snapshot_state && (allow_state || docs[i].state_root) && !state_off) {
            std::vector<uint8_t> o2, vv2, roots2;
            lmsnap::StateBase sb;
            if (lmsnap::snapshot_state_to_updates(p, l, o2, vv2, &roots2, docs[i].state_root != 0, &sb)) {
              st_hist[i].emplace_back(p, p + l);
              conv.push_back(std::move(o2)); p = conv.back().data(); l = conv.back().size();
              froot.resize(h_froot_off[i]); froot.insert(froot.end(), roots2.begin(), roots2.end());
              vvo_tmp[i].resize(8);
              for (int x = 0; x < 8; x++) vvo_tmp[i][x] = (uint8_t)(sb.synth_peer >> (8 * x));
              vvo_tmp[i].insert(vvo_tmp[i].end(), vv2.begin(), vv2.end());
              n_state_docs++;
              bsrc[b] = p; blen[b] = l;
              continue;
            }
          }
          std::vector<uint8_t> o, roots;
          size_t n_changes = 0;
          int st = lmsnap::snapshot_to_updates(p, l, o, &roots, &n_changes);
          if (st == lmsnap::SN_OK) {
            conv.push_back(std::move(o)); p = conv.back().data(); l = conv.back().size();
            if (!have_snapshot || n_changes > best_changes) { froot.resize(h_froot_off[i]); froot.insert(froot.end(), roots.begin(), roots.end()); best_changes = n_changes; have_snapshot = true; }
          }
          else if (st == lmsnap::SN_CHECKSUM) { p = stub_checksum; l = 22; }
          else if (st == lmsnap::SN_DECODE) { p = stub_decode; l = 22; }
        }
        bsrc[b] = p; blen[b] = l;
      }
    }
    h_vvo.clear(); h_vvo_off.assign(nd + 1, 0);
    for (size_t i = 0; i < nd; i++) { h_vvo_off[i] = h_vvo.size(); h_vvo.insert(h_vvo.end(), vvo_tmp[i].begin(), vvo_tmp[i].end()); }
    h_vvo_off[nd] = h_vvo.size();
    if (n_state_docs) {
      b_vvo.ensure(h_vvo.size() + 16); lmbe::h2d(b_vvo.p, h_vvo.data(), h_vvo.size());
      b_vvo_off.ensure((nd + 1) * 8); lmbe::h2d(b_vvo_off.p, h_vvo_off.data(), (nd + 1) * 8);
    }
    for (size_t i = 0; i < nd; i++) if (docs[i].n == 0) h_froot_off[i] = froot.size();
    h_froot_off[nd] = froot.size();
    for (size_t i = nd; i-- > 0;) if (h_froot_off[i] > h_froot_off[i + 1]) h_froot_off[i] = h_froot_off[i + 1];
    b_froot.ensure(froot.size() + 16); if (!froot.empty()) lmbe::h2d(b_froot.p, froot.data(), froot.size());
    b_froot_off.ensure((nd + 1) * 8); lmbe::h2d(b_froot_off.p, h_froot_off.data(), (nd + 1) * 8);
    bool direct = kn.stage_direct && nb > 0 && conv.empty();
    if (direct) {
      uint64_t sum = 0;
      for (size_t j = 0; j < nb && direct; j++) {
        sum += blen[j];
        if (((uintptr_t)bsrc[j] & 15) || (j && bsrc[j] < bsrc[j - 1] + blen[j - 1])) direct = false;
      }
      const uint64_t span = direct ? (uint64_t)(bsrc[nb - 1] + blen[nb - 1] - bsrc[0]) : 0;
      if (direct && (span > 2 * sum + (1u << 20) || !host_regions().find(bsrc[0], (size_t)span, nullptr))) direct = false;
    }
    staged_direct = direct;
    b = 0;
    for (size_t i = 0; i < nd; i++)
      for (size_t k = 0; k < docs[i].n; k++, b++) {
        if (blen[b] > 0xfffffff0ull) throw std::runtime_error("blob larger than 4 GiB");
        if (direct) off = (uint64_t)(bsrc[b] - bsrc[0]);
        h_blob_off[b] = off;
        h_blob_len[b] = (uint32_t)blen[b];
        h_blob_doc[b] = (uint32_t)i;
        in_bytes += blen[b];
        off += (blen[b] + 15) & ~(uint64_t)15;
      }
    h_blob_off[nb] = off;
    data_bytes = off + 64;
    if (!direct && data_bytes > h_stage_cap) {
      if (h_stage) lmbe::hfree(h_stage);
      h_stage_cap = data_bytes + data_bytes / 4 + 4096;
      h_stage = (uint8_t*)lmbe::halloc(h_stage_cap);
      if (!h_stage) { h_stage_cap = 0; throw std::runtime_error("host staging allocation failed"); }
    }
    b_data.ensure(data_bytes);
    st_base = direct ? bsrc[0] : h_stage;
    if (direct) {
      const uint64_t span = (uint64_t)(bsrc[nb - 1] + blen[nb - 1] - bsrc[0]);
      uint64_t CHUNK = 64ull << 20;
      for (uint64_t o = 0; o < span; o += CHUNK) lmbe::h2d_async((uint8_t*)b_data.p + o, bsrc[0] + o, span - o < CHUNK ? span - o : CHUNK);
// ... 365 lines not shown
    lmbe::tic(profiling);
    {
      std::vector<uint32_t> big;
      for (uint32_t i = 0; i < n_blobs; i++) if (h_blob_len[i] >= BIG_BLOB) big.push_back(i);
      std::stable_sort(big.begin(), big.end(), [&](uint32_t a, uint32_t b) { return h_blob_len[a] > h_blob_len[b]; });
      b_blob_hash.ensure((size_t)n_blobs * 4 + 4);
      d.blob_hash = b_blob_hash.as<uint32_t>();
      if (!big.empty()) {
        b_big.ensure(big.size() * 4);
        lmbe::h2d(b_big.p, big.data(), big.size() * 4);
        LM_LAUNCH(k_hash_big_blobs, cdiv(big.size(), HASH_G), 64, d, (const uint32_t*)b_big.as<uint32_t>(), (uint32_t)big.size());
      }
    }
    if (n_blobs) LM_LAUNCH(k_frame_count, cdiv(n_blobs, 64), 64, d);
    lmbe::toc("k_frame_count", times, profiling);
    scan(d.blob_nblk, d.blob_blk0, n_blobs, 1);
    lmbe::d2h(&NB, d.blob_blk0 + n_blobs, 4);
    d.n_blocks = NB;
    b_blk.ensure((size_t)(NB + 1) * sizeof(BlockDesc));
    b_bcnt.ensure((size_t)(NB + 1) * BCN * 4);
    b_boff.ensure((size_t)(NB + 1) * BCN * 4);
    d.blk = b_blk.as<BlockDesc>();
    d.bcnt = b_bcnt.as<uint32_t>();
    d.boff = b_boff.as<uint32_t>();
    lmbe::tic(profiling);
    if (n_blobs) LM_LAUNCH(k_frame_fill, cdiv(n_blobs, 64), 64, d);
    if (NB) LM_LAUNCH(k_block_desc, cdiv(NB, 64), 64, d);
    b_tot.ensure(64 * 4);
    d.dec_stat = b_tot.as<uint32_t>() + 48; d.dec_slot = kn.dec_slot; d.cut_min_rows = kn.cut_min_rows; d.vs_row_cost = kn.vs_row_cost;
    lmbe::dmemset(d.dec_stat, 0, 12);
    n_fused = 0;
    h_fused.assign(n_docs, 0);
    const bool mf_on = kn.map_fused && kn.redo && kn.lww_lds && kn.ht_opt && kn.ht_opt <= LWW_LDS_CAP && !resident && st_valid && NB;
    if (mf_on) {
      b_blk_kind.ensure((size_t)(NB + 1) * 4); b_doc_fused.ensure((size_t)n_docs + 16);
      d.blk_kind = b_blk_kind.as<uint32_t>();
      LM_LAUNCH(k_block_kind, cdiv(NB, 64), 64, d);
      LM_LAUNCH(k_doc_kind, cdiv(n_docs, 64), 64, d, b_doc_fused.as<uint8_t>(), kn.mf_min_rows, kn.mf_chg_ratio);
      d.doc_fused = b_doc_fused.as<uint8_t>();
    }
    if (NB) LM_LAUNCH(k_block_count, cdiv(NB, 64), 64, d);
    lmbe::toc("k_frame_fill+k_block_count", times, profiling);
    scan(d.bcnt, d.boff, NB, BCN);
    uint32_t tot[BCN];
    lmbe::d2h(tot, d.boff + (uint64_t)NB * BCN, sizeof tot);
    if (mf_on) { lmbe::d2h(h_fused.data(), b_doc_fused.p, n_docs); for (uint32_t i = 0; i < n_docs; i++) n_fused += h_fused[i]; }
    if (!n_fused) d.doc_fused = nullptr;
    const uint32_t NF = n_fused ? tot[BC_MAPOP] : 0u;
    const uint32_t KF = n_fused * LWW_LDS_CAP;
    uint32_t dec_stat[3] = {0, 0, 0};
    lmbe::d2h(dec_stat, d.dec_stat, 12);
    uint32_t ND = tot[BC_DEP], NK = tot[BC_KEY];
    NC = tot[BC_CHG]; NO = tot[BC_OP]; NCID = tot[BC_CID]; NP = tot[BC_PEER];
    b_chg.ensure((size_t)(NC + 1) * sizeof(ChangeRow));
    b_dep_peer.ensure((size_t)(ND + 1) * 4); b_dep_ctr.ensure((size_t)(ND + 1) * 4); b_dep_ci.ensure((size_t)(ND + 1) * 4);
    if ((uint64_t)NO + NF > 0xfffffff0ull || (uint64_t)NK + KF > 0xfffffff0ull) throw std::runtime_error("batch too large for 32-bit row indices");
    b_op.ensure((size_t)(NO + NF + 1) * sizeof(OpRow)); b_op_val.ensure((size_t)(NO + NF + 1) * 8); b_op_blk.ensure((size_t)(NO + NF + 1) * 4);
    b_key_off.ensure((size_t)(NK + KF + 1) * 8); b_key_len.ensure((size_t)(NK + KF + 1) * 4);
    d.n_op_rows = NO; sv_NK = NK;
    b_cid_raw.ensure((size_t)(NCID + 1) * 16); b_cid_map.ensure((size_t)(NCID + 1) * 4);
    b_peer_raw.ensure((size_t)(NP + 1) * 8); b_peer_map.ensure((size_t)(NP + 1) * 4);
    b_doc.ensure((size_t)n_docs * sizeof(DocMeta));
    b_peer_uniq.ensure((size_t)(NP + 1) * 8);
    for (DBuf* b : {&b_peer_end, &b_peer_ext, &b_peer_base, &b_peer_end_all, &b_elem_base, &b_peer_chg0, &b_peer_chg1}) b->ensure((size_t)(NP + 1) * 4);
    b_cont.ensure((size_t)(NCID + 1) * sizeof(ContRow));
    for (DBuf* b : {&b_chg_sorted, &b_chg_lamport, &b_chg_skip, &b_chg_flag, &b_node_first, &b_node_last, &b_node_order, &b_chg_node,
                    &b_node_done, &b_node_lam})
      b->ensure((size_t)(NC + 1) * 4);
    b_blk_sorted.ensure((size_t)(NB + 1) * 4);
    b_chg_mask.ensure((size_t)(NC + 1) * 8);
    b_cont_root0.ensure((size_t)(NCID + 1) * 4); b_cont_nroot.ensure((size_t)(NCID + 1) * 4);
    d.chg = b_chg.as<ChangeRow>(); d.dep_peer = b_dep_peer.as<uint32_t>(); d.dep_ctr = b_dep_ctr.as<uint32_t>(); d.dep_ci = b_dep_ci.as<uint32_t>();
    d.op = b_op.as<OpRow>(); d.op_val = b_op_val.as<uint64_t>(); d.op_blk = b_op_blk.as<uint32_t>();
    d.key_off = b_key_off.as<uint64_t>(); d.key_len = b_key_len.as<uint32_t>();
    d.cid_raw = b_cid_raw.as<uint32_t>(); d.cid_map = b_cid_map.as<uint32_t>();
    d.peer_raw = b_peer_raw.as<uint64_t>(); d.peer_map = b_peer_map.as<uint32_t>();
    d.doc = b_doc.as<DocMeta>(); d.peer_uniq = b_peer_uniq.as<uint64_t>();
    d.peer_end = b_peer_end.as<uint32_t>(); d.peer_ext = b_peer_ext.as<uint32_t>(); d.peer_base = b_peer_base.as<uint32_t>(); d.peer_end_all = b_peer_end_all.as<uint32_t>(); d.elem_base = b_elem_base.as<uint32_t>();
    d.peer_chg0 = b_peer_chg0.as<uint32_t>(); d.peer_chg1 = b_peer_chg1.as<uint32_t>();
    d.cont = b_cont.as<ContRow>();
    d.chg_sorted = b_chg_sorted.as<uint32_t>(); d.chg_lamport = b_chg_lamport.as<uint32_t>();
    d.chg_skip = b_chg_skip.as<uint32_t>(); d.chg_flag = b_chg_flag.as<uint32_t>(); d.chg_mask = b_chg_mask.as<uint32_t>();
    d.node_first = b_node_first.as<uint32_t>(); d.node_last = b_node_last.as<uint32_t>(); d.node_order = b_node_order.as<uint32_t>();
    d.cont_root0 = b_cont_root0.as<uint32_t>(); d.cont_nroot = b_cont_nroot.as<uint32_t>();
    g.blk_sorted = b_blk_sorted.as<uint32_t>(); g.chg_node = b_chg_node.as<uint32_t>();
    g.node_done = b_node_done.as<uint32_t>(); g.node_lam = b_node_lam.as<uint32_t>();
    lmbe::dmemset(b_chg_flag.p, 0, (size_t)(NC + 1) * 4);
    lmbe::dmemset(b_chg_mask.p, 0, (size_t)(NC + 1) * 8);
    lmbe::dmemset(b_chg_skip.p, 0, (size_t)(NC + 1) * 4);
    lmbe::dmemset(b_chg_lamport.p, 0, (size_t)(NC + 1) * 4);
    lmbe::tic(profiling);
    if (NB) {
#if defined(LM_PROF_DEC) || defined(LM_PROF_DAG)
      b_prof.ensure((size_t)n_docs * 16 * 8); d.prof = b_prof.as<unsigned long long>(); lmbe::dmemset(b_prof.p, 0, (size_t)n_docs * 16 * 8);
#endif
      if (n_fused) LM_LAUNCH(k_block_head, cdiv(NB, 64), 64, d);
      if (n_fused == n_docs) {}
      else if (!kn.decode_wave) LM_LAUNCH(k_block_decode, cdiv(NB, 64), 64, d);
      else {
        uint32_t slot_cap = kn.dec_slot;
        uint32_t slot_big = 0;
        if (dec_stat[0] && kn.dec_slot_big && (kn.dec_big_mode == 2 || (uint64_t)dec_stat[0] * 10 >= (uint64_t)NB * 9)) {
          if (kn.dec_big_mode == 2) { slot_big = (dec_stat[1] + 15u) & ~15u; if (slot_big > kn.dec_slot_big) slot_big = kn.dec_slot_big; }
          else { slot_big = (dec_stat[2] + 15u) & ~15u; if (slot_big < 64) slot_big = 64; if (slot_big >= slot_cap) slot_big = 0; }
        }
        if (!(slot_big && dec_stat[0] == NB))
          LM_LAUNCH_DYN(k_block_decode_wave, cdiv(NB, DEC_G), 64, (size_t)DEC_G * slot_cap + DEC_LDS_FIXED + DEC_G * DEC_KINDS, d, slot_cap, 0u, slot_big ? slot_cap : 0xffffffffu);
        if (slot_big) LM_LAUNCH_DYN(k_block_decode_wave_map, cdiv(NB, DEC_G), 64, (size_t)DEC_G * slot_big + DEC_LDS_FIXED + DEC_G * DEC_KINDS, d, slot_big, slot_cap, 0xffffffffu);
      }
      if (kn.reclass) LM_LAUNCH(k_block_reclassify, cdiv(NB, 64), 64, d);
    }
    lmbe::toc("k_block_decode", times, profiling);
    lmbe::tic(profiling);
    LM_LAUNCH(k_doc_ranges, cdiv(n_docs, 64), 64, d);
    LM_LAUNCH(k_doc_tables, n_docs, 64, d);
    uint32_t nmax = NO > NC ? NO : NC;
    if (nmax) LM_LAUNCH(k_remap, cdiv(nmax, 256), 256, d, NO, NC);
    lmbe::toc("k_doc_tables+k_remap", times, profiling);
    lmbe::tic(profiling);
    LM_LAUNCH(k_dag_a, n_docs, 64, d, g);
    lmbe::toc("k_dag_a", times, profiling);
    h_doc.resize(n_docs);
    lmbe::d2h(h_doc.data(), d.doc, (size_t)n_docs * sizeof(DocMeta));
    if (span && !resident && kn.span_auto) {
      uint64_t rows_all = 0, rows_common = 0, atoms_common = 0;
      uint32_t rows_max = 0, elems_max = 0;
      for (uint32_t i = 0; i < n_docs; i++) {
        const DocMeta& m = h_doc[i];
        if (m.status != ST_OK) continue;
        const bool checked_out = h_front_off.size() > i + 1 && h_front_off[i + 1] > h_front_off[i];
        rows_all += m.n_op;
        if (!(m.flags & DF_PLAIN) || checked_out || !plain_on) { rows_common += m.n_op; atoms_common += m.atoms; }
        rows_max = m.n_op > rows_max ? m.n_op : rows_max;
        elems_max = m.n_elems > elems_max ? m.n_elems : elems_max;
      }
      if (rows_all && rows_max < 4096 && elems_max < 65536 && rows_common * 2 >= rows_all && atoms_common < 3 * rows_common) {
        span = false; DIR_CAP_MAX = 36000u; plain_mode = 0; plain_on = false;
      }
    }
    d.span = span ? 1u : 0u;
    d.res_vis = resident ? 1u : 0u;
    uint64_t elem = 0, leaves = 0, vvh = 0;
    h_ht0.assign(n_docs, 0); h_ht_cap.assign(n_docs, 0); h_ht_full.assign(n_docs, 0);
    for (uint32_t i = 0; i < n_docs; i++) {
      DocMeta& m = h_doc[i];
      bool ok = m.status == ST_OK;
      if (!plain_on || !ok || (!resident && h_front_off.size() > i + 1 && h_front_off[i + 1] > h_front_off[i])) m.flags &= ~(DF_PLAIN | DF_FUSED);
      if (resident || plain_mode != 2 || !kn.fuse_rows) m.flags &= ~DF_FUSED;
      any_plain |= (m.flags & DF_PLAIN) != 0;
      any_fused |= (m.flags & DF_FUSED) != 0;
      want_dcnt |= ok && !(m.flags & (DF_PLAIN | DF_MOVABLE));
      m.elem0_lo = (uint32_t)elem; m.elem0_hi = (uint32_t)(elem >> 32);
      if (resident) {
        uint64_t need = (uint64_t)m.atoms + m.atoms / 2 + 68ull * (m.n_peers + 1) + 8;
        if (ok && need > tk_elem_cap[i]) {
          uint64_t cap = ((need + need / 2 + 80ull * 8) + 15) & ~15ull;
          if (cap > 0xfffffff0ull) throw std::runtime_error("resident element slice beyond 32-bit indices");
          tk_elem0[i] = elem_top; tk_elem_cap[i] = (uint32_t)cap; elem_top += cap;
        }
        m.elem0_lo = (uint32_t)tk_elem0[i]; m.elem0_hi = (uint32_t)(tk_elem0[i] >> 32);
      }
      uint32_t lc = ok ? m.n_elems / 32 + 2 * m.n_cont + 2 : 0;
      if (ok && span) {
        uint64_t items = 3ull * m.n_op + 2ull * m.n_nodes * m.n_peers + 64;
        uint64_t lcs = items / 32 + 2 * m.n_cont + 2;
        if (lcs < lc) lc = (uint32_t)lcs;
      }
      if (leaves + lc > 0xfffffff0ull) throw std::runtime_error("batch too large for 32-bit pool indices");
      m.leaf0 = (uint32_t)leaves; m.leaf_cap = lc;
      if (resident) {
        if (ok && lc > tk_leaf_cap[i]) {
          uint32_t cap = lc + lc / 2 + 8;
          if ((uint64_t)leaf_top + cap > 0xfffffff0ull) throw std::runtime_error("resident leaf pool beyond 32-bit indices");
          tk_leaf0[i] = leaf_top; tk_leaf_cap[i] = cap; leaf_top += cap; tk_reset[i] = 1;
        }
        m.leaf0 = tk_leaf0[i]; m.leaf_cap = ok ? tk_leaf_cap[i] : 0;
        if (ok && (tk_pcap[i] == 0 || m.n_peers > tk_pcap[i] || m.n_cont > tk_ccap[i])) tk_grow(i, m.n_peers, m.n_cont);
      }
      m.vvh0_lo = (uint32_t)vvh; m.vvh0_hi = (uint32_t)(vvh >> 32);
      if (ok) { elem += ((uint64_t)m.atoms + 15) & ~15ull; leaves += lc; vvh += (uint64_t)m.n_nodes * m.n_peers; }
      if (ok && m.leaf_cap > dir_cap) dir_cap = m.leaf_cap;
      uint32_t lo = ok ? m.n_elems / 40 + 2 * m.n_cont + 16 : 0;
      if (ok && span) { uint32_t los = (uint32_t)((3ull * m.n_op / 2) / 40) + 2 * m.n_cont + 16; if (los < lo) lo = los; }
      if (lo > lc) lo = lc;
      if (lo > dir_opt) dir_opt = lo;
      if (ok && m.n_peers > pmax) pmax = m.n_peers;
      uint32_t cap = 0;
      if (ok && m.n_mapop) { cap = 64; while (cap < 2 * m.n_mapop) cap <<= 1; }
      h_ht_full[i] = cap;
      if (kn.ht_opt && !resident && !(m.flags & DF_MOVABLE) && cap > kn.ht_opt) cap = kn.ht_opt;
      h_ht0[i] = ht; h_ht_cap[i] = cap;
      ht += cap;
    }
    if (resident) tk_flush();
    if (dir_cap > DIR_CAP_MAX) dir_cap = DIR_CAP_MAX;
    {
      std::vector<uint32_t> order(n_docs);
      for (uint32_t i = 0; i < n_docs; i++) order[i] = i;
      std::stable_sort(order.begin(), order.end(), [&](uint32_t a, uint32_t b) { return h_doc[a].n_op > h_doc[b].n_op; });
      b_order.ensure((size_t)n_docs * 4 + 4);
      lmbe::h2d(b_order.p, order.data(), (size_t)n_docs * 4);
      d.doc_order = b_order.as<uint32_t>();
    }
    lmbe::h2d(d.doc, h_doc.data(), (size_t)n_docs * sizeof(DocMeta));
    if (resident) {
      b_cp.ensure_keep((elem_top + 1) * 4, b_cp.cap); b_loc.ensure_keep((elem_top + 4) * 4, b_loc.cap); b_dcnt.ensure((elem_top + 1) * 4); b_tb.ensure_keep(elem_top + 16, b_tb.cap);
      b_it.ensure_keep(((size_t)leaf_top + 1) * SP_REC * 4, b_it.cap);
      for (DBuf* b : {&b_dir_out, &b_dir_out2, &b_dir_b, &b_dir_b2}) b->ensure_keep(((size_t)leaf_top + 1) * 4, b->cap);
    } else {
      b_cp.ensure((elem + 1) * 4); b_loc.ensure((elem + 4) * 4); b_tb.ensure(elem + 16);
      if (LM_BATCH_VSWEEP && want_dcnt && span && kn.version_sweep) b_dcnt.ensure((elem + 1) * 4);
      b_it.ensure((leaves + 1) * (span ? (size_t)SP_REC : 256) * 4);
      b_dir_out.ensure((leaves + 1) * 4);
    }
    b_lf_chunk.ensure(leaves + 64);
    b_vvh.ensure((vvh + 1) * 4);
    b_prof.ensure((size_t)n_docs * 16 * 8);
    d.prof = b_prof.as<unsigned long long>();
#if !defined(LM_PROF_DEC) && !defined(LM_PROF_DAG)
    lmbe::dmemset(b_prof.p, 0, (size_t)n_docs * 16 * 8);
#endif
    b_ht_key.ensure((ht + 1) * 8); b_ht_best.ensure((ht + 1) * 8); b_ht_pfx.ensure((ht + 1) * 8); b_ht_list.ensure((ht + 1) * 8);
    b_ht0.ensure((size_t)n_docs * 8); b_ht_cap.ensure((size_t)n_docs * 4); b_ht_cnt.ensure((size_t)n_docs * 4 + 4);
    lmbe::h2d(b_ht0.p, h_ht0.data(), (size_t)n_docs * 8);
    lmbe::h2d(b_ht_cap.p, h_ht_cap.data(), (size_t)n_docs * 4);
    d.cp = b_cp.as<uint32_t>(); d.loc = b_loc.as<uint32_t>(); d.dcnt = ((resident || (LM_BATCH_VSWEEP && want_dcnt && span)) && kn.version_sweep) ? b_dcnt.as<uint32_t>() : nullptr; d.tb = b_tb.as<uint8_t>();
    d.it = b_it.as<uint32_t>();
    d.dir_out = b_dir_out.as<uint32_t>();
    d.lf_chunk = b_lf_chunk.as<uint8_t>();
    d.vvh = b_vvh.as<uint32_t>();
    d.ht_key = b_ht_key.as<unsigned long long>(); d.ht_best = b_ht_best.as<unsigned long long>(); d.ht_pfx = b_ht_pfx.as<unsigned long long>();
    d.ht0 = b_ht0.as<uint64_t>(); d.ht_cap = b_ht_cap.as<uint32_t>();
    d.ht_list = b_ht_list.as<uint32_t>(); d.ht_cnt = b_ht_cnt.as<uint32_t>();
    lmbe::dmemset(b_ht_cnt.p, 0, (size_t)n_docs * 4 + 4);
    d.loc_cleared = (!resident && span && kn.loc_memset) ? 1u : 0u;
    d.no_linear = kn.linear && !keep_tombstones ? 0u : 1u;
    d.posdel_redo = (kn.redo && kn.posdel && st_valid && (resident ? shared_mode != 0 : !span)) ? 1u : 0u;
    d.posdel_off = nullptr; d.pd_row_idx = nullptr;
    if (span && !resident && kn.posdel) {
      uint64_t pieces = 0;
      bool big = false;
      std::vector<uint64_t> h_pd_off(n_docs + 1);
      for (uint32_t i = 0; i < n_docs; i++) {
        h_pd_off[i] = pieces;
        const bool on_state = n_state_docs && h_vvo_off.size() > (size_t)i + 1 && h_vvo_off[i + 1] > h_vvo_off[i] && h_doc[i].n_op > PD_CAP / 2;
        pieces += on_state ? (uint64_t)kn.pd_state_pieces * h_doc[i].n_op + PD_CAP + 1 : (uint64_t)PD_CAP;
        big |= on_state;
      }
      h_pd_off[n_docs] = pieces;
      b_posdel.ensure((size_t)pieces * 3 * 4 + 16); d.posdel = b_posdel.as<uint32_t>();
      if (big) {
        b_pd_off.ensure(((size_t)n_docs + 1) * 8); lmbe::h2d(b_pd_off.p, h_pd_off.data(), ((size_t)n_docs + 1) * 8);
        b_pd_row.ensure(((size_t)NO + 1) * 4); lmbe::dmemset(b_pd_row.p, 0xff, ((size_t)NO + 1) * 4);
        d.posdel_off = b_pd_off.as<uint64_t>(); d.pd_row_idx = b_pd_row.as<uint32_t>();
      }
    }
    if (d.loc_cleared && elem) {
      const uint64_t n4 = ((uint64_t)elem + 3) / 4;
      const uint32_t blocks = (uint32_t)std::min<uint64_t>((n4 + 255) / 256, 4096);
      LM_LAUNCH(k_fill_words, blocks, 256, b_loc.as<uint32_t>(), n4, NONE, blocks * 256u);
    }
    if (ht) { lmbe::dmemset(b_ht_key.p, 0xff, ht * 8); lmbe::dmemset(b_ht_best.p, 0, ht * 8); }
      if (resident) {
        sv.d = d; sv.g = g; sv.NB = NB; sv.NC = NC; sv.NO = NO; sv.NCID = NCID; sv.NP = NP; sv.ht = ht;
        sv.dir_cap = dir_cap; sv.dir_opt = dir_opt; sv.pmax = pmax; sv.h_doc = h_doc;
      }
    }
    lmbe::dmemset(b_cont_root0.p, 0, (size_t)(NCID + 1) * 4);
    lmbe::dmemset(b_cont_nroot.p, 0, (size_t)(NCID + 1) * 4);
    DevRes rs;
    memset(&rs, 0, sizeof rs);
    if (resident) {
      upload_res();
      rs.doc = b_res.as<ResDoc>(); rs.tk = b_tk.as<uint32_t>();
      if (!reuse) {
        h_old_blobs.resize(n_docs);
        for (uint32_t i = 0; i < n_docs; i++) h_old_blobs[i] = (uint32_t)r_blobs[i].size() - r_step[i];
        b_old_blobs.ensure((size_t)n_docs * 4 + 4);
        lmbe::h2d(b_old_blobs.p, h_old_blobs.data(), (size_t)n_docs * 4);
        d.res_old_blobs = b_old_blobs.as<uint32_t>();
        sv.d.res_old_blobs = d.res_old_blobs;
      }
      if (!reuse) { b_elem_cap.ensure((size_t)(NP + 1) * 4); d.elem_cap = b_elem_cap.as<uint32_t>(); sv.d.elem_cap = d.elem_cap; }
      LM_LAUNCH(k_res_layout, n_docs, 64, d, rs);
    }
    lmbe::tic(profiling);
    d.fuse = nullptr;
    if (!resident && any_fused && NO) {
      b_fuse.ensure(((size_t)NO + 1) * 8);
      d.fuse = b_fuse.as<uint32_t>();
      LM_LAUNCH(k_fuse_rows, cdiv(NO, 256), 256, d, NO);
    }
    if (!resident) LM_LAUNCH(k_dag_b, n_docs, 64, d, g, 0u);
    else {
      if (!reuse) {
        LM_LAUNCH(k_dag_b, n_docs, 64, d, g, 1u);
        b_doc_saved.ensure((size_t)n_docs * sizeof(DocMeta));
        lmbe::d2d(b_doc_saved.p, b_doc.p, (size_t)n_docs * sizeof(DocMeta));
      }
      LM_LAUNCH(k_dag_b, n_docs, 64, d, g, 2u);
    }
    lmbe::toc("k_dag_b", times, profiling);
    if (resident) {
      std::vector<uint64_t> loff(n_docs + 1, 0);
      for (uint32_t i = 0; i < n_docs; i++) { uint64_t N = h_doc[i].status == ST_OK ? h_doc[i].n_nodes : 0; loff[i + 1] = loff[i] + 3 * (8 * N + 64) + 3 * (4 * N + 64) + N + 16; }
      b_lca_off.ensure((size_t)(n_docs + 1) * 8); lmbe::h2d(b_lca_off.p, loff.data(), (size_t)(n_docs + 1) * 8);
      b_lca_scratch.ensure((loff[n_docs] + 16) * 4);
      b_lca_out.ensure((size_t)n_docs * LCA_OUT * 4 + 16);
      DevLca lc;
      lc.out = b_lca_out.as<uint32_t>(); lc.scratch = b_lca_scratch.as<uint32_t>(); lc.scratch_off = b_lca_off.as<uint64_t>();
      lc.prev_doc = have_prev ? b_prev_doc.as<DocMeta>() : nullptr; lc.prev_uniq = b_prev_uniq.as<uint64_t>(); lc.prev_end = b_prev_end.as<uint32_t>();
      lmbe::tic(profiling);
      LM_LAUNCH(k_import_lca, n_docs, 64, d, g, lc);
      lmbe::toc("k_import_lca", times, profiling);
    }
    lmbe::tic(profiling);
    bool any_elems = resident;
    for (uint32_t i = 0; i < n_docs && !any_elems; i++) any_elems = h_doc[i].status == ST_OK && h_doc[i].n_elems != 0;
    if (NB && !reuse && any_elems) LM_LAUNCH(k_elem_fill, NB, 64, d);
    lmbe::toc("k_elem_fill", times, profiling);
    lmbe::tic(profiling);
    b_tot.ensure(64 * 4);
    uint32_t* retry_cnt = b_tot.as<uint32_t>() + 32;
    lmbe::dmemset(retry_cnt, 0, 16);
    if (n_fused && ht && !reuse) {
      std::vector<uint32_t> mfd, mfk(n_docs, 0);
      uint32_t rank = 0;
      for (uint32_t i = 0; i < n_docs; i++) if (h_fused[i]) { mfk[i] = sv_NK + rank * LWW_LDS_CAP; rank++; if (h_doc[i].status == ST_OK && h_doc[i].n_mapop) mfd.push_back(i); }
      std::stable_sort(mfd.begin(), mfd.end(), [&](uint32_t a, uint32_t b) { return h_doc[a].n_op > h_doc[b].n_op; });
      b_mf_docs.ensure(mfd.size() * 4 + 4); b_mf_key0.ensure((size_t)n_docs * 4 + 4);
      if (!mfd.empty()) lmbe::h2d(b_mf_docs.p, mfd.data(), mfd.size() * 4);
      lmbe::h2d(b_mf_key0.p, mfk.data(), (size_t)n_docs * 4);
      DevMf mf; mf.docs = b_mf_docs.as<uint32_t>(); mf.doc_fused = d.doc_fused; mf.key0 = b_mf_key0.as<uint32_t>(); mf.stop_after = 0;
      if (const char* e = getenv("LM_MF_STOP")) mf.stop_after = (uint32_t)atoi(e);
      if (!mfd.empty()) LM_LAUNCH_DYN(k_map_fused, (uint32_t)mfd.size(), MF_WG, (size_t)MF_LDS, d, mf, retry_cnt);
    }
    if (NO && ht) {
      bool any_lds = false, any_hbm = false;
      for (uint32_t i = 0; i < n_docs; i++) if (h_doc[i].status == ST_OK && h_doc[i].n_mapop && !h_fused[i]) {
        if (kn.lww_lds && !resident && h_ht_cap[i] <= LWW_LDS_CAP && !(h_doc[i].flags & DF_MOVABLE)) any_lds = true; else any_hbm = true;
      }
      if (any_lds) LM_LAUNCH_DYN(k_map_lww_doc, n_docs, LWW_WG, (size_t)LWW_LDS_CAP * 24 + (MAX_PEERS + MAX_CONTAINERS / 32 + 8) * 4, d, retry_cnt);
      if (any_hbm) LM_LAUNCH(k_map_lww, cdiv(NO, 256), 256, d, NO, retry_cnt, 0u, any_lds ? 1u : 0u);
    }
    lmbe::toc("k_map_lww", times, profiling);
    lmbe::tic(profiling);
    dir_cap = (dir_cap + 3) & ~3u;
    dir_opt = (dir_opt + 3) & ~3u;
    if (dir_opt > DIR_CAP_MAX) dir_opt = DIR_CAP_MAX;
    size_t lds_pad = kn.lds_pad;
    if (kn.no_opt_dir) dir_opt = dir_cap;
    if (kn.dir_opt_max) { uint32_t mx = kn.dir_opt_max; if (mx >= 4 && mx < dir_opt) dir_opt = mx & ~3u; }
    const size_t dir_words = span ? 2 : 1;
    bool any_ml = false, any_common = false;
    if (resident) any_plain = false;
    for (uint32_t i = 0; i < n_docs; i++) if (h_doc[i].status == ST_OK) {
      uint32_t fl = h_doc[i].flags;
      if (resident && (fl & DF_PLAIN) && h_front_off[i + 1] > h_front_off[i]) fl &= ~DF_PLAIN;
      any_ml |= (fl & DF_MOVABLE) != 0; any_common |= (fl & (DF_MOVABLE | DF_PLAIN)) == 0;
      if (resident) any_plain |= (fl & (DF_MOVABLE | DF_PLAIN)) == DF_PLAIN;
    }
    if (resident) {
      DBuf& wa = dir_parity ? b_dir_out2 : b_dir_out; DBuf& ra = dir_parity ? b_dir_out : b_dir_out2;
      DBuf& wb = dir_parity ? b_dir_b2 : b_dir_b;     DBuf& rb = dir_parity ? b_dir_b : b_dir_b2;
      d.dir_out = wa.as<uint32_t>(); rs.dir_a_prev = ra.as<uint32_t>(); rs.dir_b = wb.as<uint32_t>(); rs.dir_b_prev = rb.as<uint32_t>();
      const size_t lds = (size_t)(2 * dir_opt + (dir_opt >> SD_BSH) + 2 + PD_LDS + 6 * pmax) * 4 + lds_pad;
      if (any_plain)
        LM_LAUNCH_DYN(k_integrate_span_res_plain, n_docs, 64, lds, d, g, dir_opt, pmax, (const OpRow*)d.op, (const ChangeRow*)d.chg, (const uint32_t*)d.chg_sorted,
                      (const uint32_t*)d.chg_skip, (const uint32_t*)d.vvh, 0u, retry_cnt, rs);
      if (any_common || !(any_ml || any_plain))
        LM_LAUNCH_DYN(k_integrate_span_res, n_docs, 64, lds, d, g, dir_opt, pmax, (const OpRow*)d.op, (const ChangeRow*)d.chg, (const uint32_t*)d.chg_sorted,
                      (const uint32_t*)d.chg_skip, (const uint32_t*)d.vvh, 0u, retry_cnt, rs);
      if (any_ml)
        LM_LAUNCH_DYN(k_integrate_span_res_ml, n_docs, 64, lds, d, g, dir_opt, pmax, (const OpRow*)d.op, (const ChangeRow*)d.chg, (const uint32_t*)d.chg_sorted,
                      (const uint32_t*)d.chg_skip, (const uint32_t*)d.vvh, 0u, retry_cnt, rs);
    } else if (span) {
      if (any_plain && plain_mode == 2) {
        LM_LAUNCH_DYN(k_integrate_span_plain_sweep, n_docs, 64, (size_t)(dir_words * dir_opt + (span ? (dir_opt >> SD_BSH) + 2 + PD_LDS : 0) + 4 * pmax + 1) * 4 + lds_pad, d, g, dir_opt, pmax, (const OpRow*)d.op,
                      (const ChangeRow*)d.chg, (const uint32_t*)d.chg_sorted, (const uint32_t*)d.chg_skip, (const uint32_t*)d.vvh, 0u, retry_cnt);
        if (d.fuse)
          LM_LAUNCH_DYN(k_integrate_span_plain_fuse, n_docs, 64, (size_t)(dir_words * dir_opt + (span ? (dir_opt >> SD_BSH) + 2 + PD_LDS : 0) + 4 * pmax + 1) * 4 + lds_pad, d, g, dir_opt, pmax, (const OpRow*)d.op,
                        (const ChangeRow*)d.chg, (const uint32_t*)d.chg_sorted, (const uint32_t*)d.chg_skip, (const uint32_t*)d.vvh, 0u, retry_cnt);
      }
      else if (any_plain)
        LM_LAUNCH_DYN(k_integrate_span_plain, n_docs, 64, (size_t)(dir_words * dir_opt + (span ? (dir_opt >> SD_BSH) + 2 + PD_LDS : 0) + 4 * pmax + 1) * 4 + lds_pad, d, g, dir_opt, pmax, (const OpRow*)d.op,
                      (const ChangeRow*)d.chg, (const uint32_t*)d.chg_sorted, (const uint32_t*)d.chg_skip, (const uint32_t*)d.vvh, 0u, retry_cnt);
      if (any_common || !(any_ml || any_plain))
        LM_LAUNCH_DYN(k_integrate_span, n_docs, 64, (size_t)(dir_words * dir_opt + (span ? (dir_opt >> SD_BSH) + 2 + PD_LDS : 0) + 4 * pmax + 1) * 4 + lds_pad, d, g, dir_opt, pmax, (const OpRow*)d.op,
                      (const ChangeRow*)d.chg, (const uint32_t*)d.chg_sorted, (const uint32_t*)d.chg_skip, (const uint32_t*)d.vvh, 0u, retry_cnt);
      if (any_ml)
        LM_LAUNCH_DYN(k_integrate_span_ml, n_docs, 64, (size_t)(dir_words * dir_opt + (span ? (dir_opt >> SD_BSH) + 2 + PD_LDS : 0) + 4 * pmax + 1) * 4 + lds_pad, d, g, dir_opt, pmax, (const OpRow*)d.op,
                      (const ChangeRow*)d.chg, (const uint32_t*)d.chg_sorted, (const uint32_t*)d.chg_skip, (const uint32_t*)d.vvh, 0u, retry_cnt);
    } else {
      LM_LAUNCH_DYN(k_integrate, n_docs, 64, (size_t)(dir_opt + 3 * pmax) * 4 + lds_pad, d, g, dir_opt, pmax, (const OpRow*)d.op,
                    (const ChangeRow*)d.chg, (const uint32_t*)d.chg_sorted, (const uint32_t*)d.chg_skip, (const uint32_t*)d.vvh, 0u, retry_cnt);
    }
    uint32_t n_retry = 0, n_lww = 0, n_posdel = 0;
    {
      uint32_t four[4] = {0, 0, 0, 0};
      lmbe::d2h(four, retry_cnt, 16);
      n_retry = four[0]; n_lww = four[2]; n_posdel = four[3];
      if (resident) last_fresh = four[1];
    }
    if (n_lww) {
      std::vector<DocMeta> hd(n_docs);
      lmbe::d2h(hd.data(), d.doc, (size_t)n_docs * sizeof(DocMeta));
      std::vector<uint32_t> h_cnt(n_docs);
      lmbe::d2h(h_cnt.data(), d.ht_cnt, (size_t)n_docs * 4);
      const uint64_t ht_old = ht;
      for (uint32_t i = 0; i < n_docs; i++) if (hd[i].flags & DF_LWW_RETRY) { h_ht0[i] = ht; h_ht_cap[i] = h_ht_full[i]; ht += h_ht_full[i]; h_cnt[i] = 0; }
      b_ht_key.ensure_keep((ht + 1) * 8, (ht_old + 1) * 8); b_ht_best.ensure_keep((ht + 1) * 8, (ht_old + 1) * 8);
      b_ht_pfx.ensure_keep((ht + 1) * 8, 0); b_ht_list.ensure_keep((ht + 1) * 8, (ht_old + 1) * 8);
      d.ht_key = b_ht_key.as<unsigned long long>(); d.ht_best = b_ht_best.as<unsigned long long>(); d.ht_pfx = b_ht_pfx.as<unsigned long long>();
// ... 603 lines not shown
```

loro_amd/csrc/lm_wave.h:

```cpp
#pragma once
#include <cstdint>
#include <cstddef>

#ifndef LM_EMU
#include <hip/hip_runtime.h>
#define LM_DEV __device__ __forceinline__
#define LM_DEV_NOINLINE __device__ __noinline__
#define LM_KERNEL extern "C" __global__
#define LM_WAVES_PER_SIMD(n) __attribute__((amdgpu_waves_per_eu(n, n)))
#define LM_SCHED_FENCE() __builtin_amdgcn_sched_barrier(0)
#define LM_ONE_WAVE_GROUPS __launch_bounds__(64)
#define LM_SHARED(type, name, n) __shared__ type name[n]
#define LM_DYN_SHARED(type, name) extern __shared__ type name[]
typedef const __attribute__((address_space(3))) uint8_t* lm_lds_bytes;

namespace lmw {
static constexpr int WAVE = 64;
LM_DEV int tid() { return (int)threadIdx.x; }
LM_DEV int bid() { return (int)blockIdx.x; }
LM_DEV int bdim() { return (int)blockDim.x; }
LM_DEV int lane() { return (int)(threadIdx.x & 63); }
LM_DEV int wave_in_block() { return (int)(threadIdx.x >> 6); }
LM_DEV void block_sync() { __syncthreads(); }
LM_DEV uint64_t ballot(bool p) { return __ballot(p); }
LM_DEV uint32_t shfl(uint32_t v, int src) { return (uint32_t)__shfl((int)v, src, 64); }
LM_DEV uint64_t shfl64(uint64_t v, int src) {
  uint32_t lo = shfl((uint32_t)v, src), hi = shfl((uint32_t)(v >> 32), src);
  return ((uint64_t)hi << 32) | lo;
}
LM_DEV uint32_t shfl_up(uint32_t v, int d) { return (uint32_t)__shfl_up((int)v, d, 64); }
LM_DEV uint32_t shfl_xor(uint32_t v, int m) { return (uint32_t)__shfl_xor((int)v, m, 64); }
LM_DEV uint32_t bcast(uint32_t v, int src) { return (uint32_t)__builtin_amdgcn_readlane((int)v, src); }
LM_DEV uint32_t first(uint32_t v) { return (uint32_t)__builtin_amdgcn_readfirstlane((int)v); }
LM_DEV uint32_t atomic_add(uint32_t* p, uint32_t v) { return atomicAdd(p, v); }
LM_DEV uint32_t atomic_min(uint32_t* p, uint32_t v) { return atomicMin(p, v); }
LM_DEV uint32_t atomic_max32(uint32_t* p, uint32_t v) { return atomicMax(p, v); }
LM_DEV void lds_add(uint32_t* p, uint32_t v) { (void)__hip_atomic_fetch_add(p, v, __ATOMIC_RELAXED, __HIP_MEMORY_SCOPE_WORKGROUP); }
LM_DEV uint64_t atomic_max64(unsigned long long* p, uint64_t v) { return atomicMax(p, (unsigned long long)v); }
LM_DEV uint32_t atomic_or(uint32_t* p, uint32_t v) { return atomicOr(p, v); }
LM_DEV uint64_t atomic_cas64(unsigned long long* p, uint64_t cmp, uint64_t v) {
  return atomicCAS(p, (unsigned long long)cmp, (unsigned long long)v);
}
LM_DEV int popc64(uint64_t m) { return __popcll(m); }
LM_DEV int ffs64(uint64_t m) { return __ffsll((unsigned long long)m) - 1; }
LM_DEV void wave_sync() { __builtin_amdgcn_wave_barrier(); }
LM_DEV void mem_fence() { __threadfence(); }
LM_DEV uint64_t clock() { return __builtin_readcyclecounter(); }
}

#else
#include <cstdio>
#include <cstdlib>
#include <cstring>
#include <vector>
#include <functional>
#include <ucontext.h>
#define LM_DEV inline
#define LM_DEV_NOINLINE inline
#define LM_KERNEL inline
#define LM_WAVES_PER_SIMD(n)
#define LM_ONE_WAVE_GROUPS
#define LM_SCHED_FENCE() do {} while (0)
#define LM_SHARED(type, name, n) static type name[n]
#define LM_DYN_SHARED(type, name) type* name = (type*)lmw::emu_dyn_shared()
typedef const uint8_t* lm_lds_bytes;

namespace lmw {
static constexpr int WAVE = 64;
#if defined(__x86_64__) && defined(__GNUC__) && !defined(LM_EMU_UCONTEXT)
struct EmuCtx { void* sp = nullptr; };
__attribute__((naked, noinline)) static void emu_switch_sp(void** , void* ) {
  __asm__ volatile(
      "pushq %rbp\n\tpushq %rbx\n\tpushq %r12\n\tpushq %r13\n\tpushq %r14\n\tpushq %r15\n\t"
      "subq $8, %rsp\n\tstmxcsr (%rsp)\n\tfnstcw 4(%rsp)\n\t"
      "movq %rsp, (%rdi)\n\tmovq %rsi, %rsp\n\t"
      "ldmxcsr (%rsp)\n\tfldcw 4(%rsp)\n\taddq $8, %rsp\n\t"
      "popq %r15\n\tpopq %r14\n\tpopq %r13\n\tpopq %r12\n\tpopq %rbx\n\tpopq %rbp\n\tret\n\t");
}
inline void emu_ctx_switch(EmuCtx* from, EmuCtx* to) { emu_switch_sp(&from->sp, to->sp); }
inline void emu_ctx_make(EmuCtx* c, char* stack, size_t size, void (*fn)()) {
  uint64_t* top = (uint64_t*)(((uintptr_t)stack + size) & ~(uintptr_t)15);
  top[-1] = 0;
  top[-2] = (uint64_t)(uintptr_t)fn;
  for (int i = 3; i <= 8; i++) top[-i] = 0;
  uint32_t* fp = (uint32_t*)(top - 9);
  fp[0] = 0x1F80;
  fp[1] = 0x037F;
  c->sp = top - 9;
}
#else
struct EmuCtx { ucontext_t uc; };
inline void emu_ctx_switch(EmuCtx* from, EmuCtx* to) { swapcontext(&from->uc, &to->uc); }
inline void emu_ctx_make(EmuCtx* c, char* stack, size_t size, void (*fn)()) {
  getcontext(&c->uc);
  c->uc.uc_stack.ss_sp = stack;
  c->uc.uc_stack.ss_size = size;
  c->uc.uc_link = nullptr;
  makecontext(&c->uc, fn, 0);
}
#endif
struct EmuFiber {
  EmuCtx ctx;
  char* stack = nullptr;
  bool done = false;
  int tid = 0;
};
struct EmuWave {
  uint64_t box[2][64];
  int arrived = 0;
  int live = 0;
  uint64_t gen = 0;
};
struct EmuBlock {
  std::vector<EmuFiber> fibers;
  std::vector<EmuWave> waves;
  EmuCtx sched;
  int cur = 0, bid = 0, bdim = 0;
  int blk_arrived = 0, blk_live = 0;
  uint64_t blk_gen = 0;
  uint64_t progress = 0;
  std::function<void()> body;
};
inline const char*& emu_kname() {
  static thread_local const char* k = "?";
  return k;
}
inline EmuBlock*& emu_cur() {
  static thread_local EmuBlock* b = nullptr;
  return b;
}
inline void emu_yield() {
  EmuBlock* b = emu_cur();
  emu_ctx_switch(&b->fibers[b->cur].ctx, &b->sched);
}
inline void emu_trampoline() {
  EmuBlock* b = emu_cur();
  b->body();
  EmuFiber& f = b->fibers[b->cur];
  f.done = true;
  EmuWave& w = b->waves[f.tid >> 6];
  w.live--;
  b->blk_live--;
  b->progress++;
  if (w.live > 0 && w.arrived == w.live) { w.arrived = 0; w.gen++; }
  if (b->blk_live > 0 && b->blk_arrived == b->blk_live) { b->blk_arrived = 0; b->blk_gen++; }
  emu_ctx_switch(&f.ctx, &b->sched);
}
inline void emu_run_block(int bid, int bdim, std::function<void()> body) {
  static const size_t STACK = 256 * 1024;
  static thread_local std::vector<char*> pool;
  EmuBlock blk;
  blk.bid = bid;
  blk.bdim = bdim;
  blk.body = body;
  blk.fibers.resize(bdim);
  blk.waves.resize((bdim + 63) / 64);
  blk.blk_live = bdim;
  EmuBlock* prev = emu_cur();
  emu_cur() = &blk;
  for (int t = 0; t < bdim; t++) {
    EmuFiber& f = blk.fibers[t];
    f.tid = t;
    if (prev) f.stack = (char*)malloc(STACK);
    else {
      if ((int)pool.size() <= t) pool.push_back((char*)malloc(STACK));
      f.stack = pool[t];
    }
    emu_ctx_make(&f.ctx, f.stack, STACK, emu_trampoline);
    blk.waves[t >> 6].live++;
  }
  int remaining = bdim;
  uint64_t last_progress = ~0ull;
  while (remaining > 0) {
    if (blk.progress == last_progress) {
      fprintf(stderr, "lm emu: deadlock in %s, workgroup %d of %d threads — lanes blocked at different collectives (non-uniform control flow)\n", emu_kname(), bid, bdim);
      abort();
    }
    last_progress = blk.progress;
    remaining = 0;
    for (int t = 0; t < bdim; t++) {
      if (blk.fibers[t].done) continue;
      blk.cur = t;
      emu_ctx_switch(&blk.sched, &blk.fibers[t].ctx);
      if (!blk.fibers[t].done) remaining++;
    }
  }
  if (prev) for (auto& f : blk.fibers) free(f.stack);
  emu_cur() = prev;
}
inline std::vector<uint64_t>& emu_dyn_buf() { static std::vector<uint64_t> v; return v; }
inline void* emu_dyn_shared() { return emu_dyn_buf().data(); }
template <class F>
inline void emu_launch(int grid, int block, size_t dyn_shared_bytes, F&& body) {
  emu_dyn_buf().assign(dyn_shared_bytes / 8 + 2, 0);
  for (int b = 0; b < grid; b++) emu_run_block(b, block, body);
}

inline int tid() { return emu_cur()->fibers[emu_cur()->cur].tid; }
inline int bid() { return emu_cur()->bid; }
inline int bdim() { return emu_cur()->bdim; }
inline int lane() { return tid() & 63; }
inline int wave_in_block() { return tid() >> 6; }
inline void block_sync() {
  EmuBlock* b = emu_cur();
  uint64_t g = b->blk_gen;
  b->blk_arrived++;
  b->progress++;
  if (b->blk_arrived == b->blk_live) { b->blk_arrived = 0; b->blk_gen++; return; }
  while (b->blk_gen == g) emu_yield();
}
inline const uint64_t* emu_exchange(uint64_t v) {
  EmuBlock* b = emu_cur();
  int t = tid();
  EmuWave& w = b->waves[t >> 6];
  uint64_t g = w.gen;
  uint64_t* box = w.box[g & 1];
  if (w.arrived == 0) memset(box, 0, sizeof(uint64_t) * 64);
  box[t & 63] = v;
  w.arrived++;
  b->progress++;
  if (w.arrived == w.live) { w.arrived = 0; w.gen++; return box; }
  while (w.gen == g) emu_yield();
  return box;
}
inline uint64_t ballot(bool p) {
  const uint64_t* x = emu_exchange(p ? 1 : 0);
  uint64_t m = 0;
  for (int i = 0; i < 64; i++) if (x[i]) m |= 1ull << i;
  return m;
}
inline uint64_t shfl64(uint64_t v, int src) {
  const uint64_t* x = emu_exchange(v);
  return x[src & 63];
}
inline uint32_t shfl(uint32_t v, int src) { return (uint32_t)shfl64(v, src); }
inline uint32_t shfl_up(uint32_t v, int d) {
  int l = lane();
  const uint64_t* x = emu_exchange(v);
  return l >= d ? (uint32_t)x[l - d] : v;
}
inline uint32_t shfl_xor(uint32_t v, int m) {
  int l = lane();
  const uint64_t* x = emu_exchange(v);
  return (uint32_t)x[(l ^ m) & 63];
}
inline uint32_t bcast(uint32_t v, int src) { return shfl(v, src); }
inline uint32_t first(uint32_t v) {
  const uint64_t* x = emu_exchange((uint64_t)v | (1ull << 32));
  for (int i = 0; i < 64; i++) if (x[i] >> 32) return (uint32_t)x[i];
  return v;
}
inline uint32_t atomic_add(uint32_t* p, uint32_t v) { uint32_t o = *p; *p = o + v; return o; }
inline uint32_t atomic_min(uint32_t* p, uint32_t v) { uint32_t o = *p; if (v < o) *p = v; return o; }
inline uint32_t atomic_max32(uint32_t* p, uint32_t v) { uint32_t o = *p; if (v > o) *p = v; return o; }
inline void lds_add(uint32_t* p, uint32_t v) { *p += v; }
inline uint64_t atomic_max64(unsigned long long* p, uint64_t v) { uint64_t o = *p; if (v > o) *p = v; return o; }
inline uint32_t atomic_or(uint32_t* p, uint32_t v) { uint32_t o = *p; *p = o | v; return o; }
inline uint64_t atomic_cas64(unsigned long long* p, uint64_t cmp, uint64_t v) { uint64_t o = *p; if (o == cmp) *p = v; return o; }
inline int popc64(uint64_t m) { return __builtin_popcountll(m); }
inline int ffs64(uint64_t m) { return m ? __builtin_ctzll(m) : -1; }
inline void wave_sync() { (void)emu_exchange(0); }
inline void mem_fence() {}
inline uint64_t clock() { return 0; }
}
#endif

#if defined(LM_EMU) && defined(LM_EMU_TRACE)
#define LM_SETERR(lhs, code) do { if (lmw::lane() == 0 || getenv("LM_EMU_ERR_ALL")) fprintf(stderr, "lm emu: " #lhs " = " #code " at %s:%d\n", __FILE__, __LINE__); (lhs) = (code); } while (0)
#else
#define LM_SETERR(lhs, code) do { (lhs) = (code); } while (0)
#endif

namespace lmw {
LM_DEV uint32_t scan_incl_add_shfl(uint32_t v) {
  int l = lane();
#pragma unroll
  for (int d = 1; d < 64; d <<= 1) {
    uint32_t t = shfl_up(v, d);
    if (l >= d) v += t;
  }
  return v;
}
#ifndef LM_EMU
LM_DEV uint32_t scan_incl_add(uint32_t v) {
  v += (uint32_t)__builtin_amdgcn_update_dpp(0, (int)v, 0x111, 0xf, 0xf, false);
  v += (uint32_t)__builtin_amdgcn_update_dpp(0, (int)v, 0x112, 0xf, 0xf, false);
  v += (uint32_t)__builtin_amdgcn_update_dpp(0, (int)v, 0x114, 0xf, 0xf, false);
  v += (uint32_t)__builtin_amdgcn_update_dpp(0, (int)v, 0x118, 0xf, 0xf, false);
  v += (uint32_t)__builtin_amdgcn_update_dpp(0, (int)v, 0x142, 0xa, 0xf, false);
  v += (uint32_t)__builtin_amdgcn_update_dpp(0, (int)v, 0x143, 0xc, 0xf, false);
  return v;
}
LM_DEV uint32_t scan_incl_max(uint32_t v) {
  uint32_t t;
  t = (uint32_t)__builtin_amdgcn_update_dpp(0, (int)v, 0x111, 0xf, 0xf, false); v = t > v ? t : v;
  t = (uint32_t)__builtin_amdgcn_update_dpp(0, (int)v, 0x112, 0xf, 0xf, false); v = t > v ? t : v;
  t = (uint32_t)__builtin_amdgcn_update_dpp(0, (int)v, 0x114, 0xf, 0xf, false); v = t > v ? t : v;
  t = (uint32_t)__builtin_amdgcn_update_dpp(0, (int)v, 0x118, 0xf, 0xf, false); v = t > v ? t : v;
  t = (uint32_t)__builtin_amdgcn_update_dpp(0, (int)v, 0x142, 0xa, 0xf, false); v = t > v ? t : v;
  t = (uint32_t)__builtin_amdgcn_update_dpp(0, (int)v, 0x143, 0xc, 0xf, false); v = t > v ? t : v;
  return v;
}
#else
LM_DEV uint32_t scan_incl_add(uint32_t v) { return scan_incl_add_shfl(v); }
LM_DEV uint32_t scan_incl_max(uint32_t v) {
  int l = lane();
  for (int d = 1; d < 64; d <<= 1) { uint32_t t = shfl_up(v, d); if (l >= d && t > v) v = t; }
  return v;
}
#endif
#ifndef LM_EMU
LM_DEV uint32_t shift_up(uint32_t v, int d) {
  uint32_t t = (uint32_t)__builtin_amdgcn_update_dpp((int)v, (int)v, 0x138, 0xf, 0xf, false);
  if (d == 2) {
    t = (uint32_t)__builtin_amdgcn_update_dpp((int)t, (int)t, 0x138, 0xf, 0xf, false);
    t = lane() < 2 ? v : t;
  }
  return t;
}
LM_DEV uint32_t shift_up0(uint32_t v, int d) {
  uint32_t t = (uint32_t)__builtin_amdgcn_mov_dpp((int)v, 0x138, 0xf, 0xf, true);
  if (d == 2) t = (uint32_t)__builtin_amdgcn_mov_dpp((int)t, 0x138, 0xf, 0xf, true);
  return t;
}
#else
LM_DEV uint32_t shift_up(uint32_t v, int d) { return shfl_up(v, d); }
LM_DEV uint32_t shift_up0(uint32_t v, int d) { uint32_t t = shfl_up(v, d); return lane() < d ? 0u : t; }
#endif
#ifndef LM_EMU
template <int N> LM_DEV uint32_t row_down(uint32_t v) { return (uint32_t)__builtin_amdgcn_mov_dpp((int)v, 0x100 | N, 0xf, 0xf, true); }
#else
template <int N> LM_DEV uint32_t row_down(uint32_t v) { int l = lane(); uint32_t t = shfl(v, (l & ~15) | ((l + N) & 15)); return (l & 15) + N > 15 ? 0u : t; }
#endif
LM_DEV uint32_t reduce_add(uint32_t v) { return bcast(scan_incl_add(v), 63); }
LM_DEV uint32_t reduce_max(uint32_t v) {
#pragma unroll
  for (int m = 32; m >= 1; m >>= 1) { uint32_t t = shfl_xor(v, m); v = t > v ? t : v; }
  return v;
}
LM_DEV uint32_t reduce_min(uint32_t v) {
#pragma unroll
  for (int m = 32; m >= 1; m >>= 1) { uint32_t t = shfl_xor(v, m); v = t < v ? t : v; }
  return v;
}
LM_DEV bool any(bool p) { return ballot(p) != 0; }
}
```

Baseline: 476,000 docs/s.

## Track valid loc slots with a per-element bitmap instead of NONE-filling loc

```diff
diff --git a/loro_amd/csrc/lm_k_decode.h b/loro_amd/csrc/lm_k_decode.h
--- a/loro_amd/csrc/lm_k_decode.h
+++ b/loro_amd/csrc/lm_k_decode.h
@@ -72,6 +72,7 @@
   uint32_t* vvh;
   uint32_t* cp;
   uint32_t* loc;
+  uint32_t* kept;
   uint32_t* dcnt;
   uint8_t* tb;
   uint32_t* it;
diff --git a/loro_amd/csrc/lm_k_integrate_span.h b/loro_amd/csrc/lm_k_integrate_span.h
--- a/loro_amd/csrc/lm_k_integrate_span.h
+++ b/loro_amd/csrc/lm_k_integrate_span.h
@@ -15,6 +15,7 @@
 struct Ts {
   uint32_t* it;
   uint32_t* loc;
+  uint32_t* kept;
   const uint32_t* ebase;
   const uint32_t* cur;
   const uint32_t* end;
@@ -90,28 +91,36 @@
 #define LM_LOC_W 64
 #endif
 static constexpr uint32_t LOC_W = LM_LOC_W;
+LM_DEV void sp_keep(Ts& t, uint32_t g, uint32_t L) {
+  t.loc[g] = L;
+  (void)lmw::atomic_or(t.kept + (g >> 5), 1u << (g & 31));
+}
 LM_DEV void sp_set_loc_lanes(Ts& t, const SpanRegs& R, bool pend, uint32_t L) {
   if (!t.loc) return;
   uint32_t len = pend ? R.len : 0u;
   uint32_t c0 = pid_ctr(R.id);
   uint32_t g = pend ? t.ebase[pid_peer(R.id)] + c0 : 0u;
-  if (pend) t.loc[g] = L;
+  if (pend) sp_keep(t, g, L);
   uint32_t k = LOC_W - (c0 & (LOC_W - 1));
-  for (uint32_t i = 0; i < 4 && lmw::any(k < len); i++, k += LOC_W) if (k < len) t.loc[g + k] = L;
+  for (uint32_t i = 0; i < 4 && lmw::any(k < len); i++, k += LOC_W) if (k < len) sp_keep(t, g + k, L);
   uint64_t m = lmw::ballot(k < len);
   while (m) {
     int j = lmw::ffs64(m);
     m &= m - 1;
     uint32_t gj = lmw::bcast(g, j), lj = lmw::bcast(len, j), kj = lmw::bcast(k, j);
-    for (uint32_t kk = kj + LOC_W * (uint32_t)lmw::lane(); kk < lj; kk += 64 * LOC_W) t.loc[gj + kk] = L;
+    for (uint32_t kk = kj + LOC_W * (uint32_t)lmw::lane(); kk < lj; kk += 64 * LOC_W) sp_keep(t, gj + kk, L);
   }
 }
 LM_DEV uint32_t ts_loc_find(const Ts& t, uint32_t pid) {
   if (!t.loc) return NONE;
   uint32_t ctr = pid_ctr(pid), lo = ctr & ~(LOC_W - 1), eb = t.ebase[pid_peer(pid)];
   uint32_t lane = (uint32_t)lmw::lane();
-  uint32_t v = (lane < LOC_W && lo + lane <= ctr) ? t.loc[eb + lo + lane] : NONE;
-  uint64_t m = lmw::ballot(v != NONE);
+  const bool in = lane < LOC_W && lo + lane <= ctr;
+  const uint32_t g = eb + lo + lane;
+  uint32_t v = in ? t.loc[g] : NONE;
+  uint32_t w = in ? lmw::load_agent(t.kept + (g >> 5)) : 0u;
+  uint64_t m = lmw::ballot(((w >> (g & 31)) & 1u) != 0);
+  lmw::emu_note_lookup(t.kept, eb + lo, LOC_W);
   if (!m) return NONE;
   int top = 63 - __builtin_clzll((unsigned long long)m);
   return lmw::bcast(v, top);
@@ -1248,10 +1257,13 @@
         nf |= !(st & ST_FUT);
         for (uint32_t k = 0; k < ln && t.loc; k++) {
 #ifdef LM_LOC16
-          uint32_t expect = (k == 0 || ((id0 + k) & (LOC_W - 1)) == 0) ? L : NONE;
-#else
-          uint32_t expect = L;
-#endif
+          const bool want = k == 0 || ((id0 + k) & (LOC_W - 1)) == 0;
+          const uint32_t gk = ts_g(t, id0 + k);
+          const bool bit = ((t.kept[gk >> 5] >> (gk & 31)) & 1u) != 0;
+          if (bit != want) { fprintf(stderr, "CHECK %s row=%u: kept bit of %u:%u is %d, expected %d (leaf %u)\n", what, row, id0 >> 24, (id0 & 0xffffff) + k, (int)bit, (int)want, L); ok = false; break; }
+          if (!bit) continue;
+#endif
+          const uint32_t expect = L;
           if (t.loc[ts_g(t, id0 + k)] != expect) { fprintf(stderr, "CHECK %s row=%u: loc of %u:%u is %u, item lives in leaf %u\n", what, row, id0 >> 24, (id0 & 0xffffff) + k, t.loc[ts_g(t, id0 + k)], L); ok = false; break; }
         }
       }
@@ -1350,14 +1362,20 @@
   if (retry_pass && m.status != (POS ? ST_POSDEL : ST_RETRY)) return;
   if (status_fatal(m.status) && !retry_pass) return;
   const bool keep_loc = RES && !ML && !retry_pass && (m.flags & DF_LAYOUT_SAME) != 0;
+  uint32_t from = 0;
+  if (keep_loc) from = lmw::first((rs.tk + rs.doc[doc].tk_off)[6]);
+#ifdef LM_LOC16
+  if (RES || !d.loc_cleared || retry_pass) {
+    uint32_t* kw = d.kept + (elem0 >> 5);
+    for (uint32_t i = (from >> 5) + (uint32_t)lane; i < (m.atoms + 31) / 32; i += 64) kw[i] = 0u;
+  }
+  if (ML)
+#endif
   {
     struct alignas(16) U4 { uint32_t x, y, z, w; };
     U4* l4 = (U4*)(d.loc + elem0);
     const U4 none4 = {NONE, NONE, NONE, NONE};
-    uint32_t from4 = 0;
-    if (keep_loc) from4 = lmw::first((rs.tk + rs.doc[doc].tk_off)[6]) / 4;
-    if (RES || !d.loc_cleared || retry_pass)
-      for (uint32_t i = from4 + (uint32_t)lane; i < (m.atoms + 3) / 4; i += 64) l4[i] = none4;
+    for (uint32_t i = from / 4 + (uint32_t)lane; i < (m.atoms + 3) / 4; i += 64) l4[i] = none4;
   }
   if (retry_pass) {
     for (uint32_t c = (uint32_t)lane; c < m.n_cont; c += 64) {
@@ -1417,6 +1435,7 @@
   Ts t;
   t.it = d.it + (uint64_t)m.leaf0 * SP_REC;
   t.loc = d.loc + elem0;
+  t.kept = d.kept + (elem0 >> 5);
   t.ebase = s_ebase; t.cur = s_cur; t.end = s_end; t.da = s_da; t.db = s_db; t.ds = s_ds; t.ds_on = false;
   t.dir_cap = dir_cap; t.leaf_cap = m.leaf_cap; t.n_leaf = 0; t.err = 0; t.beyond = 0;
   t.n_alive = 0;
@@ -1859,7 +1878,7 @@
     }
     lmw::mem_fence();
     lmw::block_sync();
-    if (lane == 0) { tk[1] = P; tk[2] = m.n_cont; tk[3] = t.n_leaf; tk[4] = m.elem0_lo; tk[5] = m.elem0_hi; tk[6] = (m.atoms + 3) & ~3u; tk[7] = m.pending_lo | m.pending_hi; tk[8] = m.atoms; tk[0] = 1; }
+    if (lane == 0) { tk[1] = P; tk[2] = m.n_cont; tk[3] = t.n_leaf; tk[4] = m.elem0_lo; tk[5] = m.elem0_hi; tk[6] = (m.atoms + 31) & ~31u; tk[7] = m.pending_lo | m.pending_hi; tk[8] = m.atoms; tk[0] = 1; }
   }
   if (lane == 0) d.doc[doc].pad0 = dir_used;
 #ifdef LM_PROF
@@ -1970,7 +1989,7 @@
     uint32_t p = p0 + (uint32_t)lane;
     bool need = p < P && s_base[p] == NONE;
     uint32_t ext = p < P ? d.peer_ext[m.praw0 + p] : 0u;
-    uint32_t cap = need ? ((ext + ext / 2 + 64 + 3) & ~3u) : 0u;
+    uint32_t cap = need ? ((ext + ext / 2 + 64 + 31) & ~31u) : 0u;
     uint32_t inc = lmw::scan_incl_add(cap);
     if (need) { s_base[p] = top + inc - cap; s_cap[p] = cap; }
     top += lmw::bcast(inc, 63);
@@ -1982,7 +2001,7 @@
       for (uint32_t p0 = 0; p0 < P; p0 += 64) {
         uint32_t p = p0 + (uint32_t)lane;
         uint32_t ext = p < P ? d.peer_ext[m.praw0 + p] : 0u;
-        uint32_t cap = p < P ? ((ext + ext / 2 + 64 + 3) & ~3u) : 0u;
+        uint32_t cap = p < P ? ((ext + ext / 2 + 64 + 31) & ~31u) : 0u;
         uint32_t inc = lmw::scan_incl_add(cap);
         if (p < P) { s_base[p] = top + inc - cap; s_cap[p] = cap; }
         top += lmw::bcast(inc, 63);
diff --git a/loro_amd/csrc/lm_k_scan.h b/loro_amd/csrc/lm_k_scan.h
--- a/loro_amd/csrc/lm_k_scan.h
+++ b/loro_amd/csrc/lm_k_scan.h
@@ -109,5 +109,9 @@
   const U4 w4 = {v, v, v, v};
   for (uint64_t i = (uint64_t)lmw::bid() * (uint64_t)lmw::bdim() + (uint64_t)lmw::tid(); i < n4; i += n_threads) q[i] = w4;
 }
+LM_KERNEL void k_fill_unkept(uint32_t* loc, const uint32_t* kept, uint64_t n, uint32_t v, uint32_t n_threads) {
+  for (uint64_t i = (uint64_t)lmw::bid() * (uint64_t)lmw::bdim() + (uint64_t)lmw::tid(); i < n; i += n_threads)
+    if (!((kept[i >> 5] >> (i & 31)) & 1u)) loc[i] = v;
+}
 
 }
diff --git a/loro_amd/csrc/lm_pipeline.h b/loro_amd/csrc/lm_pipeline.h
--- a/loro_amd/csrc/lm_pipeline.h
+++ b/loro_amd/csrc/lm_pipeline.h
@@ -91,7 +91,7 @@
   DBuf b_doc, b_peer_uniq, b_peer_end, b_peer_ext, b_peer_base, b_peer_end_all, b_elem_base, b_peer_chg0, b_peer_chg1, b_cont;
   DBuf b_chg_mask, b_chg_sorted, b_chg_lamport, b_chg_skip, b_chg_flag, b_node_first, b_node_last, b_node_order, b_vvh;
   DBuf b_blk_sorted, b_chg_node, b_node_done, b_node_lam;
-  DBuf b_cp, b_loc, b_tb, b_fuse, b_dcnt, b_posdel;
+  DBuf b_cp, b_loc, b_kept, b_tb, b_fuse, b_dcnt, b_posdel;
   DBuf b_it, b_dir_out, b_lf_chunk;
   DBuf b_cont_root0, b_cont_nroot;
   DBuf b_ht_key, b_ht_pfx, b_ht_best, b_ht0, b_ht_cap, b_ht_list, b_ht_cnt;
@@ -163,7 +163,7 @@
     std::vector<DocMeta> h_doc;
   } sv;
 
-  struct Knobs { bool span = true, decode_wave = true, no_opt_dir = false, loc_memset = true; int plain = 2; uint32_t dec_slot = 1264, dec_slot_big = 4096, dec_big_mode = 1, dir_opt_max = 0; size_t lds_pad = 0; long long slab_cap = -1; uint32_t ht_opt = 2048, cut_min_rows = 2048, vs_row_cost = 300; bool lww_lds = true, fuse_rows = true, version_sweep = true, span_auto = true, linear = true, posdel = true, reclass = true, redo = true, map_fused = true, snapshot_state = true, snapshot_state_force = false, stage_direct = true; uint32_t mf_min_rows = 2048, mf_chg_ratio = 4, pd_state_pieces = 2; } kn;
+  struct Knobs { bool span = true, decode_wave = true, no_opt_dir = false, loc_memset = true, loc_poison = false; int plain = 2; uint32_t dec_slot = 1264, dec_slot_big = 4096, dec_big_mode = 1, dir_opt_max = 0; size_t lds_pad = 0; long long slab_cap = -1; uint32_t ht_opt = 2048, cut_min_rows = 2048, vs_row_cost = 300; bool lww_lds = true, fuse_rows = true, version_sweep = true, span_auto = true, linear = true, posdel = true, reclass = true, redo = true, map_fused = true, snapshot_state = true, snapshot_state_force = false, stage_direct = true; uint32_t mf_min_rows = 2048, mf_chg_ratio = 4, pd_state_pieces = 2; } kn;
   void read_knobs() {
     Knobs k;
     if (const char* e = getenv("LM_SPAN")) k.span = atoi(e) != 0;
@@ -176,6 +176,7 @@
     if (const char* e = getenv("LM_LDS_PAD")) k.lds_pad = (size_t)atoi(e);
     k.no_opt_dir = getenv("LM_NO_OPT_DIR") != nullptr;
     if (const char* e = getenv("LM_LOC_MEMSET")) k.loc_memset = atoi(e) != 0;
+    if (const char* e = getenv("LM_LOC_POISON")) k.loc_poison = atoi(e) != 0;
     if (const char* e = getenv("LM_DIR_OPT_MAX")) k.dir_opt_max = (uint32_t)atoi(e);
     if (const char* e = getenv("LM_SLAB_CAP")) k.slab_cap = atoll(e);
     if (const char* e = getenv("LM_HT_OPT")) k.ht_opt = (uint32_t)atoi(e);
@@ -272,7 +273,7 @@
                    &b_vvo, &b_vvo_off, &b_blk, &b_bcnt, &b_boff, &b_blk_kind, &b_doc_fused, &b_mf_docs, &b_mf_key0, &b_chg, &b_dep_peer, &b_dep_ctr, &b_dep_ci, &b_op, &b_op_val, &b_op_blk, &b_key_off, &b_key_len,
                    &b_cid_raw, &b_cid_map, &b_peer_raw, &b_peer_map, &b_doc, &b_peer_uniq, &b_peer_end, &b_peer_ext, &b_peer_base, &b_peer_end_all, &b_elem_base,
                    &b_peer_chg0, &b_peer_chg1, &b_cont, &b_chg_mask, &b_chg_sorted, &b_chg_lamport, &b_chg_skip, &b_chg_flag, &b_node_first,
-                   &b_node_last, &b_node_order, &b_vvh, &b_blk_sorted, &b_chg_node, &b_node_done, &b_node_lam, &b_cp, &b_loc, &b_tb, &b_it,
+                   &b_node_last, &b_node_order, &b_vvh, &b_blk_sorted, &b_chg_node, &b_node_done, &b_node_lam, &b_cp, &b_loc, &b_kept, &b_tb, &b_it,
                    &b_dir_out, &b_lf_chunk, &b_fuse, &b_dcnt, &b_posdel, &b_pd_off, &b_pd_row,
                    &b_cont_root0, &b_cont_nroot, &b_prof, &b_hash, &b_order, &b_ht_key, &b_ht_pfx, &b_ht_best, &b_ht0, &b_ht_cap, &b_ht_list, &b_ht_cnt, &b_slab, &b_vslab, &b_slab_off, &b_vslab_off, &b_slab2, &b_slab2_off, &b_out, &b_out_off,
                    &b_vv_out, &b_vv_off, &b_tk, &b_res, &b_dir_out2, &b_dir_b, &b_dir_b2, &b_doc_saved, &b_elem_cap, &b_old_blobs, &b_prev_doc, &b_prev_uniq, &b_prev_end, &b_lca_out, &b_lca_scratch, &b_lca_off};
@@ -944,9 +945,9 @@
       want_dcnt |= ok && !(m.flags & (DF_PLAIN | DF_MOVABLE));
       m.elem0_lo = (uint32_t)elem; m.elem0_hi = (uint32_t)(elem >> 32);
       if (resident) {
-        uint64_t need = (uint64_t)m.atoms + m.atoms / 2 + 68ull * (m.n_peers + 1) + 8;
+        uint64_t need = (uint64_t)m.atoms + m.atoms / 2 + 96ull * (m.n_peers + 1) + 8;
         if (ok && need > tk_elem_cap[i]) {
-          uint64_t cap = ((need + need / 2 + 80ull * 8) + 15) & ~15ull;
+          uint64_t cap = ((need + need / 2 + 80ull * 8) + 31) & ~31ull;
           if (cap > 0xfffffff0ull) throw std::runtime_error("resident element slice beyond 32-bit indices");
           tk_elem0[i] = elem_top; tk_elem_cap[i] = (uint32_t)cap; elem_top += cap;
         }
@@ -970,7 +971,7 @@
         if (ok && (tk_pcap[i] == 0 || m.n_peers > tk_pcap[i] || m.n_cont > tk_ccap[i])) tk_grow(i, m.n_peers, m.n_cont);
       }
       m.vvh0_lo = (uint32_t)vvh; m.vvh0_hi = (uint32_t)(vvh >> 32);
-      if (ok) { elem += ((uint64_t)m.atoms + 15) & ~15ull; leaves += lc; vvh += (uint64_t)m.n_nodes * m.n_peers; }
+      if (ok) { elem += ((uint64_t)m.atoms + 31) & ~31ull; leaves += lc; vvh += (uint64_t)m.n_nodes * m.n_peers; }
       if (ok && m.leaf_cap > dir_cap) dir_cap = m.leaf_cap;
       uint32_t lo = ok ? m.n_elems / 40 + 2 * m.n_cont + 16 : 0;
       if (ok && span) { uint32_t los = (uint32_t)((3ull * m.n_op / 2) / 40) + 2 * m.n_cont + 16; if (los < lo) lo = los; }
@@ -996,11 +997,11 @@
     }
     lmbe::h2d(d.doc, h_doc.data(), (size_t)n_docs * sizeof(DocMeta));
     if (resident) {
-      b_cp.ensure_keep((elem_top + 1) * 4, b_cp.cap); b_loc.ensure_keep((elem_top + 4) * 4, b_loc.cap); b_dcnt.ensure((elem_top + 1) * 4); b_tb.ensure_keep(elem_top + 16, b_tb.cap);
+      b_cp.ensure_keep((elem_top + 1) * 4, b_cp.cap); b_loc.ensure_keep((elem_top + 4) * 4, b_loc.cap); b_kept.ensure_keep((elem_top / 32 + 4) * 4, b_kept.cap); b_dcnt.ensure((elem_top + 1) * 4); b_tb.ensure_keep(elem_top + 16, b_tb.cap);
       b_it.ensure_keep(((size_t)leaf_top + 1) * SP_REC * 4, b_it.cap);
       for (DBuf* b : {&b_dir_out, &b_dir_out2, &b_dir_b, &b_dir_b2}) b->ensure_keep(((size_t)leaf_top + 1) * 4, b->cap);
     } else {
-      b_cp.ensure((elem + 1) * 4); b_loc.ensure((elem + 4) * 4); b_tb.ensure(elem + 16);
+      b_cp.ensure((elem + 1) * 4); b_loc.ensure((elem + 4) * 4); b_kept.ensure((elem / 32 + 4) * 4); b_tb.ensure(elem + 16);
       if (LM_BATCH_VSWEEP && want_dcnt && span && kn.version_sweep) b_dcnt.ensure((elem + 1) * 4);
       b_it.ensure((leaves + 1) * (span ? (size_t)SP_REC : 256) * 4);
       b_dir_out.ensure((leaves + 1) * 4);
@@ -1016,7 +1017,7 @@
     b_ht0.ensure((size_t)n_docs * 8); b_ht_cap.ensure((size_t)n_docs * 4); b_ht_cnt.ensure((size_t)n_docs * 4 + 4);
     lmbe::h2d(b_ht0.p, h_ht0.data(), (size_t)n_docs * 8);
     lmbe::h2d(b_ht_cap.p, h_ht_cap.data(), (size_t)n_docs * 4);
-    d.cp = b_cp.as<uint32_t>(); d.loc = b_loc.as<uint32_t>(); d.dcnt = ((resident || (LM_BATCH_VSWEEP && want_dcnt && span)) && kn.version_sweep) ? b_dcnt.as<uint32_t>() : nullptr; d.tb = b_tb.as<uint8_t>();
+    d.cp = b_cp.as<uint32_t>(); d.loc = b_loc.as<uint32_t>(); d.kept = b_kept.as<uint32_t>(); d.dcnt = ((resident || (LM_BATCH_VSWEEP && want_dcnt && span)) && kn.version_sweep) ? b_dcnt.as<uint32_t>() : nullptr; d.tb = b_tb.as<uint8_t>();
     d.it = b_it.as<uint32_t>();
     d.dir_out = b_dir_out.as<uint32_t>();
     d.lf_chunk = b_lf_chunk.as<uint8_t>();
@@ -1048,9 +1049,15 @@
       }
     }
     if (d.loc_cleared && elem) {
-      const uint64_t n4 = ((uint64_t)elem + 3) / 4;
+      const uint64_t n4 = ((uint64_t)elem / 32 + 3) / 4;
       const uint32_t blocks = (uint32_t)std::min<uint64_t>((n4 + 255) / 256, 4096);
-      LM_LAUNCH(k_fill_words, blocks, 256, b_loc.as<uint32_t>(), n4, NONE, blocks * 256u);
+      LM_LAUNCH(k_fill_words, blocks, 256, b_kept.as<uint32_t>(), n4, 0u, blocks * 256u);
+    }
+    if (kn.loc_poison && span && (resident ? elem_top : elem)) {
+      const uint64_t n = resident ? elem_top : elem, n4 = (n + 3) / 4;
+      const uint32_t blocks = (uint32_t)std::min<uint64_t>(((resident ? n : n4) + 255) / 256, 4096);
+      if (resident) LM_LAUNCH(k_fill_unkept, blocks, 256, b_loc.as<uint32_t>(), b_kept.as<uint32_t>(), n, 0u, blocks * 256u);
+      else LM_LAUNCH(k_fill_words, blocks, 256, b_loc.as<uint32_t>(), n4, 0u, blocks * 256u);
     }
     if (ht) { lmbe::dmemset(b_ht_key.p, 0xff, ht * 8); lmbe::dmemset(b_ht_best.p, 0, ht * 8); }
       if (resident) {
diff --git a/loro_amd/csrc/lm_wave.h b/loro_amd/csrc/lm_wave.h
--- a/loro_amd/csrc/lm_wave.h
+++ b/loro_amd/csrc/lm_wave.h
@@ -38,6 +38,7 @@
 LM_DEV void lds_add(uint32_t* p, uint32_t v) { (void)__hip_atomic_fetch_add(p, v, __ATOMIC_RELAXED, __HIP_MEMORY_SCOPE_WORKGROUP); }
 LM_DEV uint64_t atomic_max64(unsigned long long* p, uint64_t v) { return atomicMax(p, (unsigned long long)v); }
 LM_DEV uint32_t atomic_or(uint32_t* p, uint32_t v) { return atomicOr(p, v); }
+LM_DEV uint32_t load_agent(const uint32_t* p) { return __hip_atomic_load(p, __ATOMIC_RELAXED, __HIP_MEMORY_SCOPE_AGENT); }
 LM_DEV uint64_t atomic_cas64(unsigned long long* p, uint64_t cmp, uint64_t v) {
   return atomicCAS(p, (unsigned long long)cmp, (unsigned long long)v);
 }
@@ -46,6 +47,7 @@
 LM_DEV void wave_sync() { __builtin_amdgcn_wave_barrier(); }
 LM_DEV void mem_fence() { __threadfence(); }
 LM_DEV uint64_t clock() { return __builtin_readcyclecounter(); }
+LM_DEV void emu_note_lookup(const uint32_t*, uint32_t, uint32_t) {}
 }
 
 #else
@@ -53,6 +55,7 @@
 #include <cstdlib>
 #include <cstring>
 #include <vector>
+#include <map>
 #include <functional>
 #include <ucontext.h>
 #define LM_DEV inline
@@ -256,12 +259,31 @@
 inline void lds_add(uint32_t* p, uint32_t v) { *p += v; }
 inline uint64_t atomic_max64(unsigned long long* p, uint64_t v) { uint64_t o = *p; if (v > o) *p = v; return o; }
 inline uint32_t atomic_or(uint32_t* p, uint32_t v) { uint32_t o = *p; *p = o | v; return o; }
+inline uint32_t load_agent(const uint32_t* p) { return *p; }
 inline uint64_t atomic_cas64(unsigned long long* p, uint64_t cmp, uint64_t v) { uint64_t o = *p; if (o == cmp) *p = v; return o; }
 inline int popc64(uint64_t m) { return __builtin_popcountll(m); }
 inline int ffs64(uint64_t m) { return m ? __builtin_ctzll(m) : -1; }
 inline void wave_sync() { (void)emu_exchange(0); }
 inline void mem_fence() {}
 inline uint64_t clock() { return 0; }
+struct EmuLookups { uint64_t n[2]; std::map<std::pair<const uint32_t*, uint32_t>, uint64_t> seen; };
+inline EmuLookups& emu_lookups() { static EmuLookups s; return s; }
+inline void emu_note_lookup(const uint32_t* bits, uint32_t slot0, uint32_t width) {
+  if (lane() != 0) return;
+  EmuLookups& s = emu_lookups();
+  uint64_t w = 0;
+  for (uint32_t i = 0; i < width; i++) w |= (uint64_t)((bits[(slot0 + i) >> 5] >> ((slot0 + i) & 31)) & 1u) << i;
+  auto key = std::make_pair(bits, slot0);
+  auto it = s.seen.find(key);
+  s.n[0]++;
+  if (it != s.seen.end() && it->second != w) s.n[1]++;
+  s.seen[key] = w;
+}
+extern "C" __attribute__((used, visibility("default"))) inline uint64_t lmemu_loc_stat(int i) {
+  EmuLookups& s = emu_lookups();
+  if (i < 0) { s.n[0] = s.n[1] = 0; s.seen.clear(); return 0; }
+  return s.n[i & 1];
+}
 }
 #endif
 
```

Result: faster. 492,200 docs/s (median of 6 runs) (+3.4%).
